# jtrefon/blt

Hardware: AMD Instinct MI355X
Metric: input GB/s tokenized (BPE) at 1/2/4/8 MI355X; % HBM roofline (higher is better)
Workload: dtype u8; 1 GPU; cfg3: 1024 MiB synthetic text per GPU, 50000-line merges, --chunksize 16MB; stream_bytes=1073741824, bytes_per_gpu=1073741824, chunk_size=16777216, merges=50000, parallelism=chunk-sharded x1, no collective

## Files before the change

blt_amd/_lib.py:

```python
from __future__ import annotations

import ctypes
import os
import re

_HERE = os.path.dirname(os.path.abspath(__file__))
LIB_PATH = os.environ.get("BLT_LIB_PATH") or os.path.join(_HERE, "libblt_bpe.so")
HEADER_PATH = os.path.join(os.path.dirname(_HERE), "include", "blt_bpe.h")

BLT_E_NOT_FOUND = -2
BLT_E_INVALID_DATA = -74
BLT_E_INVALID_INPUT = -22
BLT_E_NOSPC = -28
BLT_E_NOMEM = -12
BLT_E_IO = -5
BLT_E_NODEV = -19

ERROR_KINDS = {
    BLT_E_NOT_FOUND: "NotFound",
    BLT_E_INVALID_DATA: "InvalidData",
    BLT_E_INVALID_INPUT: "InvalidInput",
    BLT_E_NOSPC: "NoSpace",
    BLT_E_NOMEM: "OutOfMemory",
    BLT_E_IO: "Other",
    BLT_E_NODEV: "NoDevice",
}


class BltError(OSError):

    def __init__(self, code: int, message: str):
        super().__init__(-code, message)
        self.code = code
        self.kind = ERROR_KINDS.get(code, "Other")
        self.message = message

    def __str__(self):
        return self.message


_lib = None

_u16p = ctypes.POINTER(ctypes.c_uint16)
_u64p = ctypes.POINTER(ctypes.c_uint64)
_szp = ctypes.POINTER(ctypes.c_size_t)
_vp = ctypes.c_void_p

class RunConfig(ctypes.Structure):
    _fields_ = [("input_path", ctypes.c_char_p), ("output_path", ctypes.c_char_p), ("bpe", ctypes.c_void_p),
                ("passthrough", ctypes.c_int), ("content_token", ctypes.c_uint32), ("threads", ctypes.c_uint64),
                ("chunk_size", ctypes.c_uint64), ("n_gpus", ctypes.c_int)]


_SIGNATURES = {
    "blt_version": (ctypes.c_char_p, []),
    "blt_last_error": (ctypes.c_char_p, []),
    "blt_load_bpe_merges": (ctypes.c_int, [ctypes.c_char_p, _u16p, _u16p, _u16p, ctypes.c_size_t, _szp]),
    "blt_parse_chunk_size": (ctypes.c_int, [ctypes.c_char_p, _u64p]),
    "blt_effective_chunk_size": (ctypes.c_uint64, [ctypes.c_int, ctypes.c_uint64, ctypes.c_uint64, ctypes.c_uint32]),
    "blt_determine_thread_count": (ctypes.c_uint64, [ctypes.c_int, ctypes.c_uint64]),
    "blt_bpe_create": (ctypes.c_int, [_u16p, _u16p, _u16p, ctypes.c_size_t, ctypes.c_uint32, ctypes.POINTER(_vp)]),
    "blt_bpe_create_from_file": (ctypes.c_int, [ctypes.c_char_p, ctypes.POINTER(_vp)]),
    "blt_bpe_destroy": (None, [_vp]),
    "blt_bpe_info": (ctypes.c_int, [_vp, _szp, ctypes.POINTER(ctypes.c_int)]),
    "blt_bpe_clear_error": (ctypes.c_int, [_vp]),
    "blt_run_tokenizer": (ctypes.c_int, [ctypes.POINTER(RunConfig)]),
    "blt_bpe_process_chunk": (ctypes.c_int, [_vp, _vp, ctypes.c_size_t, _vp, ctypes.c_size_t, _szp]),
    "blt_bpe_process_chunks": (ctypes.c_int, [_vp, _vp, ctypes.c_size_t, ctypes.c_size_t, ctypes.c_int, _vp,
                                              ctypes.c_size_t, _szp, _vp]),
    "blt_basic_process_chunk": (ctypes.c_int, [_vp, ctypes.c_size_t, _vp, ctypes.c_size_t, _szp]),
    "blt_bpe_workspace_size": (ctypes.c_size_t, [_vp, ctypes.c_uint64, ctypes.c_uint64]),
    "blt_bpe_encode_device": (ctypes.c_int, [_vp, _vp, ctypes.c_uint64, ctypes.c_uint64, _vp, _vp, _vp,
                                             ctypes.c_size_t, _vp, _u64p]),
    "blt_bpe_encode_device_ex": (ctypes.c_int, [_vp, _vp, ctypes.c_uint64, ctypes.c_uint64, _vp, _vp, _vp,
                                                ctypes.c_size_t, _vp, _u64p, ctypes.c_uint32]),
    "blt_bpe_workspace_reset": (ctypes.c_int, [_vp, _vp, ctypes.c_uint64, ctypes.c_uint64, _vp]),
    "blt_bpe_check_workspace": (ctypes.c_int, [_vp, _vp]),
    "blt_basic_encode_device": (ctypes.c_int, [_vp, ctypes.c_uint64, _vp, _vp]),
}

_DEBUG_SIGNATURES = {
    "blt_debug_inject_device_error": (ctypes.c_int, [_vp, _vp, _vp]),
    "blt_debug_set_tile_record": (None, [_vp]),
    "blt_debug_set_inject": (ctypes.c_uint32, [ctypes.c_uint32]),
    "blt_debug_last_u16_passes": (ctypes.c_uint32, []),
    "blt_debug_last_scan_passes": (ctypes.c_uint32, []),
    "blt_debug_set_u16_chain": (ctypes.c_int, [ctypes.c_int]),
    "blt_debug_set_fused_only": (ctypes.c_int, [ctypes.c_int]),
    "blt_debug_set_shared_contexts": (None, [ctypes.c_int]),
    "blt_debug_set_pin_ring": (ctypes.c_int, [ctypes.c_int]),
    "blt_debug_set_fused": (None, [ctypes.c_int]),
    "blt_debug_last_fused": (ctypes.c_uint32, []),
    "blt_debug_byte_mode": (ctypes.c_int, [_vp]),
    "blt_debug_chain_depth": (ctypes.c_uint32, [_vp]),
    "blt_debug_set_finish": (ctypes.c_int, [ctypes.c_int]),
    "blt_debug_set_sparse": (ctypes.c_int, [ctypes.c_int]),
    "blt_debug_last_sparse": (ctypes.c_uint32, []),
    "blt_debug_set_sparse_cap": (ctypes.c_uint32, [ctypes.c_uint32]),
    "blt_debug_available_cpus": (ctypes.c_uint64, [ctypes.c_char_p, ctypes.c_char_p, ctypes.c_uint64]),
}


def header_symbols():
    with open(HEADER_PATH) as f:
        text = f.read()
    return sorted(set(re.findall(r"\b(blt_[a-z0-9_]+)\s*\(", text)))


def _share_torch_runtime():
    if os.environ.get("BLT_STANDALONE_HIP") == "1":
        return
    try:
        import torch
        import torch.cuda
        libdir = os.path.join(os.path.dirname(torch.__file__), "lib")
        hip = os.path.join(libdir, "libamdhip64.so")
        if os.path.exists(hip):
            ctypes.CDLL(hip, mode=ctypes.RTLD_GLOBAL)
    except ImportError:
        pass


def lib():
    global _lib
    if _lib is None:
        if not os.path.exists(LIB_PATH):
            raise RuntimeError(f"{LIB_PATH} is not built: run `make` (or __graft_entry__.build())")
        _share_torch_runtime()
        L = ctypes.CDLL(LIB_PATH)
        for name, (res, args) in list(_SIGNATURES.items()) + list(_DEBUG_SIGNATURES.items()):
            try:
                fn = getattr(L, name)
            except AttributeError:
                if name in _DEBUG_SIGNATURES:
                    continue
                raise
            fn.restype = res
            fn.argtypes = args
        _lib = L
    return _lib


def check(rc: int) -> None:
    if rc != 0:
        msg = lib().blt_last_error().decode("utf-8", "replace")
        raise BltError(rc, msg)
```

blt_amd/csrc/blt_host.cpp:

```cpp
#include <errno.h>
#include <fcntl.h>
#include <sched.h>
#include <hip/hip_runtime.h>
#include <stdarg.h>
#include <stdint.h>
#include <stdio.h>
#include <string.h>
#include <unistd.h>

#include <algorithm>
#include <atomic>
#include <condition_variable>
#include <memory>
#include <mutex>
#include <string>
#include <thread>
#include <unordered_map>
#include <unordered_set>
#include <vector>

#include "../../include/blt_bpe.h"
#include "bpe_kernels.h"

namespace {
// ... 346 lines not shown
        is_comp[kv.first >> 16] = 1;
        is_comp[kv.first & 0xFFFF] = 1;
    }
    for (int t = 0; t < 65536 && h->single_pass; ++t)
        if (is_value[t] && is_comp[t]) h->single_pass = false;
    if (!h->single_pass) h->chain_depth = chain_depth(map);

    std::vector<uint8_t> used(65536, 0);
    size_t byte_pairs = 0;
    for (const auto& kv : map)
        if ((kv.first >> 16) < 256 && (kv.first & 0xFFFF) < 256) { used[kv.second] = 1; ++byte_pairs; }
    if (byte_pairs == 65536) {
        h->sentinel = 0x10000u;
    } else {
        uint32_t s = 0xFFFF;
        while (used[s]) --s;
        h->sentinel = s;
    }
    h->dense.assign(65536, (uint16_t)(h->sentinel & 0xFFFF));
    for (const auto& kv : map) {
        const uint32_t a = kv.first >> 16, b = kv.first & 0xFFFF;
        if (a < 256 && b < 256) h->dense[blt::dense_index(a, b)] = kv.second;
    }
    auto bswap = [](uint32_t v) { return (uint16_t)(((v & 0xFF) << 8) | ((v >> 8) & 0xFF)); };
    bool hi_merge = true, self_valued = false, byte_keys = true;
    std::vector<uint8_t> hi_used(256, 0);
    for (const auto& kv : map) {
        const uint32_t a = kv.first >> 16, b = kv.first & 0xFFFF;
        if (a < 256 && b < 256) {
            if (a == b) h->byte_self_pair = true;
            if (kv.second == a) self_valued = true;
            if (kv.second < 256) hi_merge = false;
            hi_used[kv.second >> 8] = 1;
        } else {
            byte_keys = false;
        }
    }
    h->allmerge = byte_pairs == 65536;
    if (hi_merge) {
        h->byte_mode = 0;
    } else if (!self_valued || h->allmerge) {
        h->byte_mode = 1;
    } else {
        h->byte_mode = -1;
        for (uint32_t m = 1; m < 256 && h->byte_mode < 0; ++m)
            if (!hi_used[m]) { h->byte_mode = 2; h->mark = m; }
    }
    h->live_first = !h->single_pass && byte_keys && h->byte_mode > 0;
    h->self_ne.assign(blt::kSelfEntries, 0);
    for (uint32_t a = 0; a < 256; ++a)
        for (uint32_t b = 0; b < 256; ++b) h->self_ne[blt::self_index(a, b)] = (uint16_t)a;
    for (const auto& kv : map) {
        const uint32_t a = kv.first >> 16, b = kv.first & 0xFFFF;
        if (a < 256 && b < 256)
            h->self_ne[blt::self_index(a, b)] = (h->byte_mode == 2 && kv.second == a) ? (uint16_t)((h->mark << 8) | a)
                                                                                     : kv.second;
    }
    h->self_be.resize(blt::kSelfEntries);
    for (uint32_t i = 0; i < blt::kSelfEntries; ++i) h->self_be[i] = bswap(h->self_ne[i]);
    if (!h->single_pass && !build_buckets(map, is_comp, h.get())) return fail(BLT_E_NOMEM, "cannot place the merge map in a hash table");
    *out = h.release();
    return 0;
}

int current_device(int* dev) {
    int count = 0;
    if (hipGetDeviceCount(&count) != hipSuccess || count < 1) return fail(BLT_E_NODEV, "no HIP device available");
    HIP_TRY(hipGetDevice(dev));
    if (*dev < 0 || *dev >= kMaxDevices) return fail(BLT_E_NODEV, "device index %d out of range", *dev);
    return 0;
}

void detail_stamp(const char* what) {
    static const bool on = getenv("BLT_CLI_TIMING") != nullptr;
    if (!on) return;
    static timespec t0 = [] { timespec t; clock_gettime(CLOCK_MONOTONIC, &t); return t; }();
    timespec t;
    clock_gettime(CLOCK_MONOTONIC, &t);
    fprintf(stderr, "blt timing: detail: %s %.4f s\n", what,
            (double)(t.tv_sec - t0.tv_sec) + 1e-9 * (double)(t.tv_nsec - t0.tv_nsec));
}

int device_tables(const blt_bpe* hc, int dev, DevTables** out, hipStream_t via = nullptr) {
    blt_bpe* h = const_cast<blt_bpe*>(hc);
    DevTables& t = h->dev[dev];
    std::call_once(t.once, [&]() {
        auto up256 = [](size_t x) { return (x + 255) & ~size_t(255); };
        const size_t b_dense = 65536 * sizeof(uint16_t), b_self = blt::kSelfEntries * sizeof(uint16_t);
        const size_t b_hash = h->hwords.size() * sizeof(uint32_t);
        const size_t o_ne = up256(b_dense), o_be = o_ne + up256(b_self), o_hash = o_be + up256(b_self);
        const size_t total = o_hash + up256(b_hash);
        std::vector<uint8_t> blob(total, 0);
        memcpy(blob.data(), h->dense.data(), b_dense);
        memcpy(blob.data() + o_ne, h->self_ne.data(), b_self);
        memcpy(blob.data() + o_be, h->self_be.data(), b_self);
        if (b_hash) memcpy(blob.data() + o_hash, h->hwords.data(), b_hash);
        hipStream_t us = via;
        uint8_t* base = nullptr;
        detail_stamp("tables: blob built");
        bool ok = us || hipStreamCreateWithFlags(&us, hipStreamNonBlocking) == hipSuccess;
        detail_stamp("tables: stream created");
        ok = ok && hipMalloc(&base, total) == hipSuccess;
        detail_stamp("tables: allocated");
        ok = ok && hipMemcpyAsync(base, blob.data(), total, hipMemcpyHostToDevice, us) == hipSuccess;
        detail_stamp("tables: copy issued");
        if (base) {
            t.dense = reinterpret_cast<uint16_t*>(base);
            t.self_ne = reinterpret_cast<uint16_t*>(base + o_ne);
            t.self_be = reinterpret_cast<uint16_t*>(base + o_be);
            if (b_hash) t.hbuckets = reinterpret_cast<uint2*>(base + o_hash);
        }
        ok = ok && hipStreamSynchronize(us) == hipSuccess;
        detail_stamp("tables: copied");
        if (us && us != via) (void)hipStreamDestroy(us);
        detail_stamp("tables: stream destroyed");
        if (!ok) t.status = BLT_E_IO;
    });
    if (t.status) return fail(t.status, "uploading merge tables to device %d failed", dev);
    *out = &t;
    return 0;
}

uint32_t* sticky_word(const blt_bpe* hc) {
    blt_bpe* h = const_cast<blt_bpe*>(hc);
    std::call_once(h->sticky_once, [h] {
        void* p = nullptr;
        if (hipHostMalloc(&p, 64, hipHostMallocMapped | hipHostMallocPortable | hipHostMallocCoherent) == hipSuccess) {
            memset(p, 0, 64);
            h->sticky.store(static_cast<uint32_t*>(p), std::memory_order_release);
        }
    });
    return h->sticky.load(std::memory_order_acquire);
}

int sticky_check(const blt_bpe* h) {
    const uint32_t* w = h->sticky.load(std::memory_order_acquire);
    if (w && __atomic_load_n(w, __ATOMIC_ACQUIRE))
        return fail(BLT_E_IO,
                    "a previous merge scan on this handle flagged a device error (look-back timeout, output range "
                    "or prefix invariant); its output is invalid (blt_bpe_clear_error resets the handle)");
    return 0;
}

uint64_t* g_debug_tiles = nullptr;
std::atomic<uint32_t> g_inject{0};
std::atomic<int> g_shared_contexts{0};
std::atomic<int> g_fused{1};
std::atomic<int> g_u16_chain{3};
std::atomic<int> g_fused_only{0};
constexpr uint32_t kEncodeNoFused = 1u << 31;
thread_local uint32_t t_last_u16_passes = 0;
thread_local uint32_t t_last_scan_passes = 0;
thread_local uint32_t t_last_fused = 0;

inline uint64_t up16(uint64_t x) { return (x + 15) & ~15ull; }
inline uint64_t up256(uint64_t x) { return (x + 255) & ~255ull; }

struct WsLayout {
    uint64_t ntiles, nchunks;
    uint64_t ctl, status, status2, total, off_a, off_b, cmap, cmap_stride, gstat, bytes, zero_bytes;
    uint64_t sp_holes, sp_bits0, sp_bits1, sp_bits2, sp_seeds0, sp_seeds1, sp_merges, sp_tileo, sp_status, sp_ctr, sp_ntiles,
        sp_slices;
    uint32_t sp_cap;
};
constexpr uint32_t kMaxBoundedPasses = 64;
inline bool chain_bounded(const blt_bpe* h) { return h->chain_depth && h->chain_depth <= kMaxBoundedPasses + 1; }
constexpr uint32_t kSparseMaxPasses = 250;
constexpr uint32_t kSparseCtrWords = 2 + 2 * (kSparseMaxPasses + 1);
constexpr uint64_t kChainBlock = 48;

WsLayout ws_layout(const blt_bpe* h, uint64_t n, uint64_t cs) {
    const bool single_pass = h->single_pass;
    WsLayout L{};
    const uint64_t tile = single_pass ? std::min<uint64_t>(blt::kTilePos, blt::kTilePosBytes)
                                      : std::min<uint64_t>(blt::kTilePosTok, blt::kTilePosBytes);
    L.ntiles = (n + tile - 1) / tile;
    L.nchunks = n ? (n + cs - 1) / cs : 0;
    L.ctl = 0;
    L.status = blt::kCtlBytes;
    L.zero_bytes = up16(blt::kCtlBytes + 8 * L.ntiles);
    L.total = L.zero_bytes;
    L.off_a = L.total + kChainBlock;
    L.off_b = L.off_a + up16(8 * (L.nchunks + 1));
    L.cmap = up256(L.off_b + up16(8 * (L.nchunks + 1)));
    L.cmap_stride = up256(8 * ((n + blt::kTokRange - 1) / blt::kTokRange));
    L.gstat = L.cmap + 3 * L.cmap_stride;
    L.status2 = up256(L.gstat + up16(8 * L.nchunks));
    L.bytes = single_pass ? L.cmap : L.status2 + up16(8 * L.ntiles);
    if (!single_pass && !chain_bounded(h) && n < (1ull << 32)) {
        const uint64_t bm = up16(4 * ((n + 31) / 32));
        const uint64_t cap = n / 16 + 4096;
        const uint64_t sptiles = (n + blt::kSparseTile - 1) / blt::kSparseTile;
        L.sp_cap = (uint32_t)cap;
        L.sp_ntiles = sptiles;
        L.sp_holes = up16(L.bytes);
        L.sp_bits0 = L.sp_holes + bm;
        L.sp_bits1 = L.sp_bits0 + bm;
        L.sp_bits2 = L.sp_bits1 + bm;
        L.sp_seeds0 = L.sp_bits2 + bm;
        L.sp_seeds1 = L.sp_seeds0 + up16(4 * cap);
        L.sp_merges = L.sp_seeds1 + up16(4 * cap);
        L.sp_tileo = L.sp_merges + up16(12 * cap);
        L.sp_status = L.sp_tileo + up16(4 * ((sptiles + 15) & ~15ull) + 16);
        L.sp_ctr = L.sp_status + up16(8 * sptiles);
        L.sp_slices = L.sp_ctr + up16(4ull * kSparseCtrWords) + 4ull * blt::kSparseSampleBlocks;
        L.bytes = L.sp_slices + 3ull * 4ull * blt::kSparseSlices;
    }
    return L;
}

int read_u64(const void* dptr, uint64_t* v, hipStream_t s) {
    HIP_TRY(hipMemcpyAsync(v, dptr, sizeof(uint64_t), hipMemcpyDeviceToHost, s));
    HIP_TRY(hipStreamSynchronize(s));
    return 0;
}

int ctl_error(const uint32_t* ctl) {
    if (ctl[1])
        return fail(BLT_E_IO,
                    "merge-scan device check failed (flags 0x%x: 1 look-back timeout, 2 output range, 4 prefix "
                    "invariant, 8 workgroup wait timeout, 16 chunk map, 32 workspace not zeroed for this size "
                    "(BLT_ENCODE_WORKSPACE_ZEROED past the last reset), 64 finish-kernel count invariant; first "
                    "at tile %u sub-tile %u, O=%llu, value=%llu, C=%u)",
                    ctl[1], ctl[2] ? ctl[2] - 1 : 0, ctl[3], (unsigned long long)ctl[4] | ((unsigned long long)ctl[5] << 32),
                    (unsigned long long)ctl[6] | ((unsigned long long)ctl[7] << 32), ctl[8]);
    return 0;
}

int check_ctl(uint8_t* ws, hipStream_t s) {
    uint32_t ctl[16] = {0};
    HIP_TRY(hipMemcpyAsync(ctl, ws, sizeof ctl, hipMemcpyDeviceToHost, s));
    HIP_TRY(hipStreamSynchronize(s));
    return ctl_error(ctl);
}

struct Chain {
    const uint64_t* n_in = nullptr;
    uint64_t* n_out = nullptr;
    uint32_t* done = nullptr;
    uint32_t pass_id = 0;
    bool next_scan = false;
};

struct U16Run {
    bool map_ready = false;
    bool st_ready = false;
    uint32_t par = 0;
    void reset() { map_ready = st_ready = false; }
};

int run_pass(const blt_bpe* h, const DevTables* t, int dev, hipStream_t s, uint8_t* ws, const WsLayout& L,
             const void* in, bool in_u16, uint64_t n, uint64_t cs, const uint64_t* cstart, void* out, bool be,
             uint64_t out_cap, uint64_t* chunk_off, bool ws_zeroed = false, const Chain* chain = nullptr,
             bool tok_scan = false, U16Run* run = nullptr) {
    const bool columnar = !in_u16 && cs >= blt::kMinChunkBytes && h->byte_mode >= 0 && be;
    const uint64_t tile = columnar ? blt::kTilePosBytes
                                   : in_u16 ? (tok_scan ? blt::kTilePosTok : blt::kTilePosU16) : blt::kTilePos;
    const uint64_t ntiles = (n + tile - 1) / tile;
    if (ntiles > 0xFFFFFFFFull) return fail(BLT_E_INVALID_INPUT, "input too large");
    if (!(g_u16_chain.load(std::memory_order_relaxed) & 1)) run = nullptr;
    const bool chained = in_u16 && chain && run;
    const bool merge_ready = chained && !tok_scan && run->st_ready;
    if (!ws_zeroed && !(in_u16 && tok_scan) && !merge_ready) {
        HIP_TRY(hipMemsetAsync(ws, 0, up16(blt::kCtlBytes + 8 * ntiles), s));
        if (chained) run->par = 0;
    }
    blt::PassParams p{};
    p.in = in;
    p.n = n;
    p.cs = cs;
    p.cstart = cstart;
    p.nchunks = L.nchunks;
    p.out = out;
    p.out_cap = out_cap;
    p.chunk_off = chunk_off;
    p.status = reinterpret_cast<uint64_t*>(ws + L.status);
    p.ctl = reinterpret_cast<uint32_t*>(ws + L.ctl);
    p.total = chain ? chain->n_out : reinterpret_cast<uint64_t*>(ws + L.total);
    if (chain) {
        p.n_dev = chain->n_in;
        p.done = chain->done;
        p.pass_id = chain->pass_id;
    }
    p.ntiles = (uint32_t)ntiles;
    p.sentinel = h->sentinel;
    p.dense = columnar ? (be ? t->self_be : t->self_ne) : t->dense;
    p.hbuckets = t->hbuckets;
    p.hmul1 = h->hmul1;
    p.hmul2 = h->hmul2;
    p.hshift = h->hshift;
    p.hbytes = (uint32_t)(h->hwords.size() * sizeof(uint32_t));
    p.hone = h->hone ? 1u : 0u;
    p.cs_magic = cs ? ~0ull / cs : 0;
    if (cs && cs % blt::kTilePosBytes == 0 && cs / blt::kTilePosBytes < (1ull << 31)) {
        p.cs_tiles = (uint32_t)(cs / blt::kTilePosBytes);
        p.cs_tiles_magic = p.cs_tiles > 1 ? (uint32_t)(0xFFFFFFFFull / p.cs_tiles) : 0u;
    }
    p.allm = h->allmerge ? 1u : 0u;
    p.mark = h->mark | (h->mark << 16);
    p.debug = g_debug_tiles;
    p.inject = g_inject.load(std::memory_order_relaxed);
    p.sticky = h->sticky.load(std::memory_order_acquire);
    const bool scan16 = in_u16 && tok_scan;
    const bool ready = scan16 && chained && run->map_ready;
    auto map = [&](uint32_t i) { return reinterpret_cast<uint64_t*>(ws + L.cmap + (uint64_t)(i % 3u) * L.cmap_stride); };
    const uint32_t r = chain ? chain->pass_id % 3u : 0u;
    if (scan16) p.cmap = map(r);
    if (chained) {
        const bool alt = run->par != 0;
        p.status = reinterpret_cast<uint64_t*>(ws + (alt ? L.status2 : L.status));
        p.status_zero = reinterpret_cast<uint64_t*>(ws + (alt ? L.status : L.status2));
        p.tick = alt ? blt::kCtlTickAlt : 0u;
        if (scan16 && chain->next_scan) {
            p.cmap_next = map(r + 1u);
            p.cmap_zero = map(r + 2u);
        }
        run->par ^= 1u;
        run->st_ready = true;
        run->map_ready = scan16 && chain->next_scan;
    }
    p.ws_check = (ws_zeroed && !in_u16 && !chain) ? 1u : 0u;
    if (columnar) HIP_TRY(blt::launch_scan_bytes(p, h->byte_mode, (chain && h->live_first) ? 1 : 0, dev, s));
    else if (scan16) {
        HIP_TRY(blt::launch_scan_tokens(p, ready ? 1 : 0, dev, s));
        ++t_last_scan_passes;
    }
    else HIP_TRY(blt::launch_merge_pass(p, in_u16 ? 1 : 0, be ? 1 : 0, dev, s));
    return 0;
}

int run_fused(const blt_bpe* h, const DevTables* t, int dev, hipStream_t s, uint8_t* ws, const WsLayout& L,
              const uint8_t* d_in, uint64_t n, uint64_t cs, uint8_t* d_out, uint64_t* chunk_off, uint64_t* total,
              uint32_t* done, uint32_t* fused_fail) {
    const uint64_t ntiles = (n + blt::kTilePosTok - 1) / blt::kTilePosTok;
    if (ntiles > 0xFFFFFFFFull) return fail(BLT_E_INVALID_INPUT, "input too large");
    blt::PassParams p{};
    p.in = d_in;
    p.n = n;
    p.cs = cs;
    p.nchunks = L.nchunks;
    p.out = d_out;
    p.out_cap = 2 * n;
    p.chunk_off = chunk_off;
    p.status = reinterpret_cast<uint64_t*>(ws + L.status);
    p.ctl = reinterpret_cast<uint32_t*>(ws + L.ctl);
    p.total = total;
    p.done = done;
    p.pass_id = 1;
    p.ntiles = (uint32_t)ntiles;
    p.hbuckets = t->hbuckets;
    p.hmul1 = h->hmul1;
    p.hmul2 = h->hmul2;
    p.hshift = h->hshift;
    p.hbytes = (uint32_t)(h->hwords.size() * sizeof(uint32_t));
    p.hone = h->hone ? 1u : 0u;
    p.cs_magic = ~0ull / cs;
    p.debug = g_debug_tiles;
    p.inject = g_inject.load(std::memory_order_relaxed);
    p.sticky = h->sticky.load(std::memory_order_acquire);
    p.fused_fail = fused_fail;
    HIP_TRY(blt::launch_scan_fused(p, dev, s));
    return 0;
}

int run_finish(const blt_bpe* h, const DevTables* t, int dev, hipStream_t s, uint8_t* ws, const WsLayout& L,
               uint8_t* d_out, uint32_t k, const uint64_t* off_in, uint64_t* off_out, uint64_t* total, uint32_t* done) {
    blt::PassParams p{};
    p.in = d_out;
    p.out = d_out;
    p.cstart = off_in;
    p.nchunks = L.nchunks;
    p.chunk_off = off_out;
    p.total = total;
    p.done = done;
    p.pass_id = k;
    p.status = reinterpret_cast<uint64_t*>(ws + L.gstat);
    p.ctl = reinterpret_cast<uint32_t*>(ws + L.ctl);
    p.hbuckets = t->hbuckets;
    p.hmul1 = h->hmul1;
    p.hmul2 = h->hmul2;
    p.hshift = h->hshift;
    p.hbytes = (uint32_t)(h->hwords.size() * sizeof(uint32_t));
    p.hone = h->hone ? 1u : 0u;
    p.sticky = h->sticky.load(std::memory_order_acquire);
    p.fin_gate = reinterpret_cast<uint32_t*>(ws + L.total + 32);
    p.debug = g_debug_tiles;
    p.inject = g_inject.load(std::memory_order_relaxed);
    HIP_TRY(blt::launch_finish(p, dev, s));
    return 0;
}

std::atomic<int> g_finish{1};

int chain_sticky(const blt_bpe* h, uint8_t* ws, const WsLayout& L, uint64_t passes) {
    if (!sticky_check(h)) return 0;
    const std::string sticky_msg = t_err;
    uint32_t ctl[16] = {0};
    if (hipMemcpy(ctl, ws + L.ctl, sizeof ctl, hipMemcpyDeviceToHost) == hipSuccess && ctl_error(ctl))
        return fail(BLT_E_IO, "%s; u16 passes 1..%llu: %s", sticky_msg.c_str(), (unsigned long long)passes, t_err.c_str());
    return fail(BLT_E_IO, "%s", sticky_msg.c_str());
}

std::atomic<int> g_sparse{1};
thread_local uint32_t t_last_sparse = 0;
std::atomic<uint32_t> g_sparse_cap{0};

struct SparseRun {
    bool gated = false;
    bool taken = false;
    bool complete = false;
    uint32_t passes = 0;
    uint32_t applied = 0;
    uint64_t rec[4] = {0, 0, 0, 0};
    bool rec_final = false;
};

struct SparseHost {
    uint32_t ctr[kSparseCtrWords];
    uint64_t rec[4];
};
struct SparseHostLease {
    const blt_bpe* h;
    SparseHost* p = nullptr;
    explicit SparseHostLease(const blt_bpe* hh) : h(hh) {
        {
            std::lock_guard<std::mutex> lk(h->sp_mu);
            if (!h->sp_free.empty()) {
                p = static_cast<SparseHost*>(h->sp_free.back());
                h->sp_free.pop_back();
            }
        }
        if (!p && hipHostMalloc(reinterpret_cast<void**>(&p), sizeof(SparseHost), hipHostMallocDefault) != hipSuccess)
            p = nullptr;
    }
    ~SparseHostLease() {
        if (!p) return;
        std::lock_guard<std::mutex> lk(h->sp_mu);
        h->sp_free.push_back(p);
    }
};

int run_sparse(const blt_bpe* h, const DevTables* t, int dev, hipStream_t s, uint8_t* ws, const WsLayout& L,
               uint8_t* d_out, const uint64_t* n_dev, uint64_t n_max, const uint64_t* gate, uint64_t k,
               const uint64_t* off_in, uint64_t* off_out, uint64_t* tot, SparseRun* r) {
    *r = SparseRun{};
    SparseHostLease lease(h);
    SparseHost* hb = lease.p;
    if (!L.sp_cap || !hb || n_max == 0 || n_max >= (1ull << 32)) return 0;
    if (dev < 0 || dev >= kMaxDevices) return fail(BLT_E_NODEV, "device index %d out of range", dev);
    uint32_t* ctr = reinterpret_cast<uint32_t*>(ws + L.sp_ctr);
    blt::SparseParams q{};
    q.tok = reinterpret_cast<uint16_t*>(d_out);
    q.n = n_max;
    q.n_dev = n_dev;
    q.gate = gate;
    q.holes = reinterpret_cast<uint32_t*>(ws + L.sp_holes);
    q.flags = ctr;
    q.merges = reinterpret_cast<uint32_t*>(ws + L.sp_merges);
    const uint32_t cap_over = g_sparse_cap.load(std::memory_order_relaxed);
    q.cap = cap_over ? std::min(cap_over, L.sp_cap) : L.sp_cap;
    q.hbuckets = t->hbuckets;
    q.hmul1 = h->hmul1;
    q.hmul2 = h->hmul2;
    q.hshift = h->hshift;
    q.hbytes = (uint32_t)(h->hwords.size() * sizeof(uint32_t));
    q.hone = h->hone ? 1u : 0u;
    q.coff_in = off_in;
    q.coff_out = off_out;
    q.nchunks = L.nchunks;
    q.tile_cnt = reinterpret_cast<uint32_t*>(ws + L.sp_tileo);
    q.super_cnt = q.tile_cnt + ((L.sp_ntiles + 15) & ~15ull);
    q.status = reinterpret_cast<uint64_t*>(ws + L.sp_status);
    q.zero = reinterpret_cast<uint4*>(ws + L.sp_tileo);
    q.zero16 = (uint32_t)(((L.sp_ctr - L.sp_tileo) + up16(4ull * kSparseCtrWords)) / 16);
    q.sample = reinterpret_cast<uint32_t*>(ws + L.sp_ctr + up16(4ull * kSparseCtrWords));
// ... 812 lines not shown
        mult = up(t[n - 2]) == 'K' ? 1024ull : 1024ull * 1024ull;
        if (num.empty()) return fail(BLT_E_INVALID_INPUT, "Number part missing for unit '%s'", t.substr(n - 2).c_str());
    } else if (digits) {
        num = t;
    } else {
        return fail(BLT_E_INVALID_INPUT,
                    "Invalid unit or format: '%s'. Number must be followed by KB, MB, or be raw bytes.", t.c_str());
    }
    uint64_t v = 0;
    if (*parse_unsigned(num, UINT64_MAX, &v)) return fail(BLT_E_INVALID_INPUT, "Invalid number: '%s'", num.c_str());
    *out = v * mult;
    return 0;
    )
}

uint64_t blt_effective_chunk_size(int has_cli, uint64_t cli, uint64_t threads, uint32_t memcap) {
    const uint64_t amin = 256ull * 1024, amax = 128ull * 1024 * 1024;
    const uint64_t dmin = 1024ull * 1024, dmax = 16ull * 1024 * 1024;
    if (has_cli) return std::min(std::max(cli, amin), amax);
    const uint64_t usable = (uint64_t)((double)total_ram_bytes() * ((double)memcap / 100.0));
    uint64_t c = usable / std::max<uint64_t>(threads, 1) / 4;
    c = std::min(std::max(c, dmin), dmax);
    return std::min(std::max(c, amin), amax);
}

uint64_t blt_determine_thread_count(int has_cli, uint64_t threads) {
    if (has_cli) return threads == 0 ? 1 : threads;
    return available_cpus();
}

int blt_bpe_create(const uint16_t* a, const uint16_t* b, const uint16_t* v, size_t n, uint32_t flags,
                   blt_bpe** out) {
    GUARDED(
    if (!out || (n && (!a || !b || !v))) return fail(BLT_E_INVALID_INPUT, "null argument");
    if (flags) return fail(BLT_E_INVALID_INPUT, "unknown flags 0x%x", flags);
    std::vector<uint32_t> keys(n);
    std::vector<uint16_t> vals(v, v + n);
    for (size_t i = 0; i < n; ++i) keys[i] = ((uint32_t)a[i] << 16) | b[i];
    return build_handle(keys, vals, out);
    )
}

int blt_bpe_create_from_file(const char* path, blt_bpe** out) {
    GUARDED(
    if (!path || !out) return fail(BLT_E_INVALID_INPUT, "null argument");
    std::vector<int32_t> table;
    if (int rc = load_merges_table(path, table)) {
        const std::string inner = t_err;
        return fail(rc, "Failed to load BPE merges: %s", inner.c_str());
    }
    std::vector<uint32_t> keys;
    std::vector<uint16_t> vals;
    for (uint32_t i = 0; i < 65536; ++i)
        if (table[i] >= 0) { keys.push_back(((i >> 8) << 16) | (i & 255)); vals.push_back((uint16_t)table[i]); }
    return build_handle(keys, vals, out);
    )
}

void blt_bpe_destroy(blt_bpe* h) {
    if (!h) return;
    for (int d = 0; d < kMaxDevices; ++d) {
        if (h->dev[d].dense) (void)hipFree(h->dev[d].dense);
    }
    if (uint32_t* w = h->sticky.load(std::memory_order_acquire)) (void)hipHostFree(w);
    for (void* p : h->sp_free) (void)hipHostFree(p);
    delete h;
}

int blt_bpe_info(const blt_bpe* h, size_t* n_entries, int* single_pass) {
    if (!h) return fail(BLT_E_INVALID_INPUT, "null handle");
    if (n_entries) *n_entries = h->n_entries;
    if (single_pass) *single_pass = h->single_pass ? 1 : 0;
    return 0;
}

int blt_bpe_clear_error(const blt_bpe* h) {
    if (!h) return fail(BLT_E_INVALID_INPUT, "null handle");
    uint32_t* w = h->sticky.load(std::memory_order_acquire);
    if (!w || !__atomic_exchange_n(w, 0u, __ATOMIC_ACQ_REL)) return 0;
    return fail(BLT_E_IO, "a merge scan on this handle had flagged a device error (now cleared)");
}

size_t blt_bpe_workspace_size(const blt_bpe* h, uint64_t n, uint64_t cs) {
    if (!h || cs == 0) return 0;
    return (size_t)ws_layout(h, n, cs).bytes;
}

int blt_bpe_encode_device(const blt_bpe* h, const uint8_t* d_in, uint64_t n, uint64_t cs, uint8_t* d_out,
                          uint64_t* d_chunk_off, void* d_ws, size_t ws_bytes, void* stream, uint64_t* out_tokens) {
    GUARDED(return encode_device(h, d_in, n, cs, d_out, d_chunk_off, d_ws, ws_bytes, (hipStream_t)stream, out_tokens);)
}

int blt_bpe_encode_device_ex(const blt_bpe* h, const uint8_t* d_in, uint64_t n, uint64_t cs, uint8_t* d_out,
                             uint64_t* d_chunk_off, void* d_ws, size_t ws_bytes, void* stream, uint64_t* out_tokens,
                             uint32_t flags) {
    if (flags & ~BLT_ENCODE_WORKSPACE_ZEROED) return fail(BLT_E_INVALID_INPUT, "unknown flags 0x%x", flags);
    GUARDED(
    return encode_device(h, d_in, n, cs, d_out, d_chunk_off, d_ws, ws_bytes, (hipStream_t)stream, out_tokens, flags);
    )
}

int blt_bpe_workspace_reset(const blt_bpe* h, void* d_ws, uint64_t n, uint64_t cs, void* stream) {
    if (!h || !d_ws || cs == 0) return fail(BLT_E_INVALID_INPUT, "bad argument");
    const WsLayout L = ws_layout(h, n, cs);
    HIP_TRY(hipMemsetAsync(d_ws, 0, L.zero_bytes, (hipStream_t)stream));
    if (L.ntiles <= 0xFFFFFFFFull)
        HIP_TRY(hipMemsetD32Async(static_cast<uint32_t*>(d_ws) + blt::kCtlCover, (int)(uint32_t)L.ntiles, 1,
                                  (hipStream_t)stream));
    return 0;
}

int blt_bpe_check_workspace(void* d_ws, void* stream) {
    if (!d_ws) return fail(BLT_E_INVALID_INPUT, "null workspace");
    hipStream_t s = (hipStream_t)stream;
    if (int rc = check_ctl(static_cast<uint8_t*>(d_ws), s)) {
        const std::string msg = t_err;
        uint32_t z[16] = {0};
        (void)hipMemcpyAsync(d_ws, z, sizeof z, hipMemcpyHostToDevice, s);
        (void)hipStreamSynchronize(s);
        return fail(rc, "%s", msg.c_str());
    }
    return 0;
}

int blt_debug_byte_mode(const blt_bpe* h) {
    if (!h) return -1;
    return (h->byte_mode & 0xFF) | (h->allmerge ? 0x100 : 0) | (h->live_first ? 0x200 : 0);
}

int blt_debug_set_finish(int on) { return g_finish.exchange(on ? 1 : 0); }
int blt_debug_set_sparse(int on) { return g_sparse.exchange(on ? 1 : 0); }
uint32_t blt_debug_last_sparse(void) { return t_last_sparse; }
uint32_t blt_debug_set_sparse_cap(uint32_t cap) { return g_sparse_cap.exchange(cap); }

uint32_t blt_debug_chain_depth(const blt_bpe* h) { return h ? h->chain_depth : 0; }

void blt_debug_set_shared_contexts(int on) { g_shared_contexts.store(on ? 1 : 0, std::memory_order_relaxed); }
int blt_debug_set_pin_ring(int on) { return g_pin_ring.exchange(on ? 1 : 0) > 0 ? 1 : 0; }

void blt_debug_set_fused(int on) { g_fused.store(on ? 1 : 0, std::memory_order_relaxed); }
int blt_debug_set_u16_chain(int bits) { return g_u16_chain.exchange(bits); }
int blt_debug_set_fused_only(int on) { return g_fused_only.exchange(on ? 1 : 0); }
uint32_t blt_debug_last_fused() { return t_last_fused; }

uint64_t blt_debug_available_cpus(const char* cgroup_root, const char* proc_cgroup, uint64_t logical) {
    return available_cpus(cgroup_root, proc_cgroup, logical);
}

void blt_debug_set_tile_record(uint64_t* d_buf) { g_debug_tiles = d_buf; }
uint32_t blt_debug_set_inject(uint32_t bits) { return g_inject.exchange(bits); }

uint32_t blt_debug_last_u16_passes(void) { return t_last_u16_passes; }
uint32_t blt_debug_last_scan_passes(void) { return t_last_scan_passes; }

int blt_debug_inject_device_error(const blt_bpe* h, void* d_ws, void* stream) {
    if (!h) return fail(BLT_E_INVALID_INPUT, "null handle");
    int dev;
    if (int rc = current_device(&dev)) return rc;
    uint32_t* w = sticky_word(h);
    if (!w) return fail(BLT_E_NOMEM, "cannot allocate the pinned error word");
    HIP_TRY(blt::launch_inject_error(static_cast<uint32_t*>(d_ws), w, (hipStream_t)stream));
    HIP_TRY(hipStreamSynchronize((hipStream_t)stream));
    return 0;
}

int blt_basic_encode_device(const uint8_t* d_in, uint64_t n, uint8_t* d_out, void* stream) {
    if ((!d_in || !d_out) && n) return fail(BLT_E_INVALID_INPUT, "null argument");
    if (((uintptr_t)d_in | (uintptr_t)d_out) & 15) return fail(BLT_E_INVALID_INPUT, "device buffers must be 16-byte aligned");
    int dev;
    if (int rc = current_device(&dev)) return rc;
    HIP_TRY(blt::launch_basic_expand(d_in, n, d_out, (hipStream_t)stream));
    return 0;
}

int blt_bpe_process_chunk(const blt_bpe* h, const uint8_t* in, size_t n, uint8_t* out, size_t out_cap,
                          size_t* out_len) {
    GUARDED(
    if (!h || !out_len || (n && (!in || !out))) return fail(BLT_E_INVALID_INPUT, "null argument");
    *out_len = 0;
    if (int rc = sticky_check(h)) return rc;
    if (n == 0) return 0;
    if (out_cap < 2 * (uint64_t)n) return fail(BLT_E_NOSPC, "out_cap %zu < 2 * n", out_cap);
    int dev;
    if (int rc = current_device(&dev)) return rc;
    uint64_t ntok = 0;
    if (int rc = encode_host_on(h, dev, in, n, n, out, &ntok, nullptr)) return rc;
    *out_len = 2 * ntok;
    return 0;
    )
}

int blt_basic_process_chunk(const uint8_t* in, size_t n, uint8_t* out, size_t out_cap, size_t* out_len) {
    GUARDED(
    if (!out_len || (n && (!in || !out))) return fail(BLT_E_INVALID_INPUT, "null argument");
    *out_len = 0;
    if (n == 0) return 0;
    if (out_cap < 2 * (uint64_t)n) return fail(BLT_E_NOSPC, "out_cap %zu < 2 * n", out_cap);
    int dev;
    if (int rc = current_device(&dev)) return rc;
    DevCtx* c = ctx_acquire(dev);
    if (!c) return fail(BLT_E_IO, "cannot create a HIP stream");
    CtxGuard guard{c};
    if (int rc = grow(&c->d_in, &c->in_cap, up16(n))) return rc;
    if (int rc = grow(&c->d_out, &c->out_cap, up16(2 * n))) return rc;
    HIP_TRY(hipMemcpyAsync(c->d_in, in, n, hipMemcpyHostToDevice, c->stream));
    HIP_TRY(blt::launch_basic_expand(c->d_in, n, c->d_out, c->stream));
    HIP_TRY(hipMemcpyAsync(out, c->d_out, 2 * n, hipMemcpyDeviceToHost, c->stream));
    HIP_TRY(hipStreamSynchronize(c->stream));
    *out_len = 2 * n;
    return 0;
    )
}

}

void blt_prewarm_chunks(const blt_bpe* h, uint64_t n, uint64_t cs, int n_gpus) try {
    if (!h || !n || !cs) return;
    const bool timing = getenv("BLT_CLI_TIMING") != nullptr;
    timespec t0;
    clock_gettime(CLOCK_MONOTONIC, &t0);
    auto stamp = [&](const char* what) {
        if (!timing) return;
        timespec t;
        clock_gettime(CLOCK_MONOTONIC, &t);
        fprintf(stderr, "blt timing: prewarm step: %s +%.4f s\n", what,
                (double)(t.tv_sec - t0.tv_sec) + 1e-9 * (double)(t.tv_nsec - t0.tv_nsec));
    };
    HostPlan plan;
    if (host_plan(h, n, cs, n_gpus, &plan) != 0) return;
    stamp("device count (runtime up)");
    const uint64_t g = plan.devs.size();
    const uint64_t nchunks = (n + cs - 1) / cs;
    const uint64_t share = (nchunks + g - 1) / g * cs;
    const uint64_t win = h->single_pass ? std::max<uint64_t>(cs, std::min<uint64_t>(kPipeWindow / cs * cs, share)) : share;
    const uint64_t per_ctx = ((n + win - 1) / win + g - 1) / g;
    const int slots = (int)std::min<uint64_t>(kPipeSlots, per_ctx);
    (void)sticky_word(h);
    detail_stamp("sticky word");
    for (uint64_t d = 0; d < g; ++d) {
        const int dev = plan.devs[d];
        if (hipSetDevice(dev) != hipSuccess) return;
        DevCtx* c = ctx_acquire(dev);
        if (!c) return;
        CtxGuard guard{c};
        stamp("context (streams)");
        DevTables* t;
        if (device_tables(h, dev, &t, c->stream) != 0) return;
        stamp("device tables");
        if (plan.multi) {
            if (slots > 0 && pipe_slot_ready(h, c->pipe[0], std::min(win, n), cs) != 0) return;
            stamp("pipeline slots");
            if (blt::launch_noop(c->pipe[0].stream) == hipSuccess) (void)hipStreamSynchronize(c->pipe[0].stream);
            stamp("code object loaded (first launch)");
        } else {
            const WsLayout L = ws_layout(h, n, cs);
            uint8_t* offp = reinterpret_cast<uint8_t*>(c->d_off);
            if (grow(&c->d_in, &c->in_cap, up16(n)) || grow(&c->d_out, &c->out_cap, up16(2 * n)) ||
                grow(&c->d_ws, &c->ws_cap, L.bytes) || grow(&offp, &c->off_cap, 8 * (L.nchunks + 1)))
                return;
            c->d_off = reinterpret_cast<uint64_t*>(offp);
        }
    }
    if (g == 1 && !plan.multi) (void)hipSetDevice(plan.devs[0]);
} catch (...) {
}

extern "C" {

int blt_bpe_process_chunks(const blt_bpe* h, const uint8_t* in, size_t n, size_t cs, int n_gpus, uint8_t* out,
                           size_t out_cap, size_t* out_len, uint64_t* chunk_out_len) {
    GUARDED(
    if (!h || !out_len || (n && (!in || !out))) return fail(BLT_E_INVALID_INPUT, "null argument");
    if (cs == 0) return fail(BLT_E_INVALID_INPUT, "chunk_size must be > 0");
    *out_len = 0;
    if (int rc = sticky_check(h)) return rc;
    if (n == 0) return 0;
    if (out_cap < 2 * (uint64_t)n) return fail(BLT_E_NOSPC, "out_cap %zu < 2 * n", out_cap);
    const uint64_t nchunks = (n + cs - 1) / cs;
    HostPlan plan;
    if (int rc = host_plan(h, n, cs, n_gpus, &plan)) return rc;
    uint64_t total = 0;
    std::vector<uint64_t> offs;
    if (!plan.multi) {
        if (int rc = encode_host_on(h, plan.devs[0], in, n, cs, out, &total, chunk_out_len ? &offs : nullptr)) return rc;
    } else {
        if (int rc = encode_host_multi(h, plan.devs, in, n, cs, out, &total, chunk_out_len ? &offs : nullptr)) return rc;
    }
    if (chunk_out_len)
        for (uint64_t k = 0; k < nchunks; ++k) chunk_out_len[k] = 2 * (offs[k + 1] - offs[k]);
    *out_len = 2 * total;
    return 0;
    )
}

}
```

blt_amd/csrc/bpe_kernels.h:

```cpp
#pragma once
#include <hip/hip_runtime.h>
#include <stdint.h>

namespace blt {

constexpr int kSub = 4;
constexpr uint64_t kTilePos = 4 * 512 * 16;
constexpr uint64_t kTilePosU16 = kTilePos;
constexpr uint64_t kTilePosTok = 32768;
constexpr uint64_t kTokRange = 1024;
constexpr uint64_t kTilePosBytes = 32768;
constexpr uint64_t kMinChunkBytes = 4096;
constexpr uint64_t kCtlBytes = 64;
constexpr uint32_t kCtlLeft = 15;
constexpr uint32_t kCtlTickAlt = 12;
constexpr uint32_t kCtlCover = 14;

struct PassParams {
    const void* in;
    uint64_t n;
    uint64_t cs;
    const uint64_t* cstart;
    uint64_t nchunks;
    void* out;
    uint64_t* chunk_off;
    uint64_t* status;
    uint32_t* ctl;
    uint64_t out_cap;
    uint64_t* total;
    uint32_t ntiles;
    uint32_t sentinel;
    const uint16_t* dense;
    const uint2* hbuckets;
    uint32_t hmul1, hmul2;
    uint32_t hshift;
    uint32_t hbytes;
    uint32_t hone;
    const uint64_t* n_dev;
    uint32_t* done;
    uint32_t pass_id;
    uint64_t* cmap;
    uint64_t* cmap_next;
    uint64_t* cmap_zero;
    uint64_t* status_zero;
    uint32_t tick;
    uint64_t cs_magic;
    uint32_t cs_tiles;
    uint32_t cs_tiles_magic;
    uint32_t allm;
    uint32_t mark;
    uint32_t* sticky;
    uint32_t* fin_gate;
    uint32_t ws_check;
    uint32_t* fused_fail;
    uint64_t* debug;
    uint32_t inject;
};
constexpr uint32_t kInjectFinish = 1u, kInjectScanTok = 2u, kInjectSparseMove = 4u;

hipError_t launch_merge_pass(const PassParams& p, int input_u16, int big_endian, int device, hipStream_t s);
hipError_t launch_scan_bytes(const PassParams& p, int mode, int live, int device, hipStream_t s);
constexpr uint32_t kDoneBytePass = 0x80000000u;
hipError_t launch_scan_tokens(const PassParams& p, int map_ready, int device, hipStream_t s);
hipError_t launch_scan_fused(const PassParams& p, int device, hipStream_t s);
hipError_t launch_finish(const PassParams& p, int device, hipStream_t s);
constexpr uint64_t kFinCapTokens = 16384;
constexpr uint32_t kFinMaxGroupChunks = 1024;
hipError_t launch_basic_expand(const uint8_t* in, uint64_t n, uint8_t* out, hipStream_t s);
hipError_t launch_chain_final(const uint64_t* tot, const uint32_t* done, const uint64_t* off1, uint64_t* chunk_off,
                              uint64_t nchunks, uint32_t k_last, uint64_t* tot_final, hipStream_t s);
struct SparseParams {
    uint16_t* tok;
    uint64_t n;
    const uint64_t* n_dev;
    const uint64_t* gate;
    const uint32_t* cond;
    uint32_t* holes;
    uint32_t* seeds_in;
    uint32_t* nseeds_in;
    const uint32_t* cnt_in;
    uint32_t* bits_in;
    uint32_t* seeds_out;
    uint32_t* nseeds_out;
    uint32_t* bits_out;
    uint32_t* bits_alt;
    uint32_t first_pass;
    uint32_t* merges;
    uint32_t* nmerges;
    uint32_t* cnt_seeds;
    uint32_t* cnt_merges;
    uint32_t slice;
    uint32_t nslices;
    uint32_t* flags;
    uint32_t cap;
    const uint2* hbuckets;
    uint32_t hmul1, hmul2, hshift;
    uint32_t hbytes, hone;
    const uint64_t* coff_in;
    uint64_t* coff_out;
    uint64_t nchunks;
    uint64_t* total;
    uint32_t* tile_cnt;
    uint32_t* super_cnt;
    uint64_t* status;
    uint32_t* ctl;
    uint32_t* sticky;
    uint32_t* sample;
    uint4* zero;
    uint32_t zero16;
    uint32_t inject;
};
constexpr uint64_t kSparseTile = 8192;
constexpr uint32_t kSparseSlices = 4096;
constexpr uint32_t kSparseSampleBlocks = 64;
constexpr uint32_t kSparseSample = kSparseSampleBlocks * 8192u;
hipError_t launch_sparse_detect(const SparseParams& q, hipStream_t s);
hipError_t launch_sparse_list(const SparseParams& q, hipStream_t s);
hipError_t launch_sparse_pass(const SparseParams& q, hipStream_t s);
hipError_t launch_sparse_compact(const SparseParams& q, const uint32_t* nseeds0, hipStream_t s);
hipError_t launch_noop(hipStream_t s);
hipError_t launch_inject_error(uint32_t* ctl, uint32_t* sticky, hipStream_t s);

inline uint32_t dense_index(uint32_t a, uint32_t b) { return (a << 8) | (b ^ ((a << 1) & 0xFEu)); }

constexpr uint32_t kSelfRow = 258;
constexpr uint32_t kSelfEntries = 256 * kSelfRow;
inline uint32_t self_index(uint32_t a, uint32_t b) { return a * kSelfRow + b; }

inline uint32_t bucket_of(uint32_t key, uint32_t mul, uint32_t shift) {
    return (uint32_t)((key & 0xFFFFu) * (mul & 0xFFFFu) + (key >> 16) * (mul >> 16)) >> shift;
}
constexpr uint32_t kHashLdsMax = 48u << 10;

}
```

blt_amd/csrc/bpe_kernels.hip:

```cpp
#include <hip/hip_runtime.h>
#include <stdint.h>

#include <stddef.h>

#include <atomic>
#include <mutex>
#include <unordered_map>

#include "bpe_kernels.h"

namespace blt {

constexpr int kThreads = 512;
constexpr int kWaves = kThreads / 64;
constexpr int kSeg = 16;
constexpr int kSubPos = kThreads * kSeg;
constexpr int kStageBytes = 2 * kSubPos + 32;
constexpr uint32_t kSpinTimeoutTicks = 20000000u;
constexpr uint32_t kSpinClockEvery = 64;
struct SpinClock {
    uint32_t t0 = 0;
    uint32_t n = 0;
    __device__ __forceinline__ bool expired() {
        if ((++n % kSpinClockEvery) != 0u) return false;
// ... 464 lines not shown
                }
                st_publish(p.status + T, st_incl(C == 1u ? co1 : co0, end));
                s_C = C; s_O = O;
                if (p.debug) {
                    uint64_t* d = p.debug + 4ull * T;
                    d[0] = O;
                    d[1] = ((uint64_t)C << 32) | how;
                    d[2] = ((uint64_t)tf.cnt1 << 32) | tf.cnt0;
                    d[3] = ((uint64_t)co1 << 32) | co0;
                }
                s_tfn[2] = tf.cnt0; s_tfn[3] = tf.cnt1;
                if (T == p.ntiles - 1) {
                    *p.total = end;
                    if (p.chunk_off) p.chunk_off[p.nchunks] = end;
                    if (!kDense && p.done && end == p.n) *p.done = p.pass_id;
                }
            }
        }
        __syncthreads();

        if (s_C > 1u) continue;
        const uint32_t C = s_C;
        const uint64_t O = s_O;
        const uint32_t tile_cnt = C ? s_tfn[3] : s_tfn[2];
#pragma unroll
        for (int j = 0; j < kSubT; ++j) {
            const uint64_t sub0 = tile0 + (uint64_t)j * kSubPos;
            const uint64_t pos = sub0 + (uint64_t)tid * kSeg;
            const int g = j * kWaves + wave;
            const uint32_t cg = s_gin[g][C];
            const uint32_t og = s_gin[g][2 + C];
            const uint32_t c = hasb[j] ? bco[j] : cg;
            const uint32_t lane_off = og + (cg ? (excl[j] >> 16) : (excl[j] & 0xFFFFu));
            const uint32_t sub_first = s_gin[j * kWaves][2 + C];
            const uint32_t sub_end = (j + 1 < kSubT) ? s_gin[(j + 1) * kWaves][2 + C] : tile_cnt;
            const uint64_t gb = 2ull * (O + sub_first), ge = 2ull * (O + sub_end);
            const uint64_t ab = gb & ~15ull;
            const uint32_t M = merges_for(mm[j], c);
            const uint32_t L = lands_for(M, c, valid[j]);
            uint16_t* st16 = reinterpret_cast<uint16_t*>(s_stage);
            uint32_t r = (uint32_t)((2ull * (O + lane_off) - ab) >> 1);
#pragma unroll
            for (int k = 0; k < 16; ++k) {
                if ((L >> k) & 1u) {
                    uint32_t v = (vals[j][k >> 1] >> (16 * (k & 1))) & 0xFFFFu;
                    if constexpr (kDense) {
                        const uint32_t tok = ((M >> k) & 1u) ? v : seg[j].at(k);
                        st16[r++] = (uint16_t)(kBE ? bswap16(tok) : tok);
                    } else {
                        st16[r++] = (uint16_t)(((M >> k) & 1u) ? v : seg[j].at(k));
                    }
                }
            }
            if (p.chunk_off && nb < (uint32_t)kThreads) {
                const uint32_t lo = (uint32_t)(pos - tile0);
                for (uint32_t a = bnd_lower(lo); a < nb; ++a) {
                    const uint32_t r = s_bnd[a];
                    if (r > lo + 15u) break;
                    const uint32_t before = __popc(L & ((1u << (r - lo)) - 1u));
                    p.chunk_off[bk0 + a] = O + lane_off + before;
                }
            } else if (p.chunk_off) {
                uint64_t kidx;
                uint64_t b = first_boundary(p, sub0 < p.n ? sub0 : p.n, kidx);
                while (b < p.n && b < sub0 + kSubPos) {
                    if (b >= pos && b < pos + 16 && kidx < p.nchunks) {
                        uint32_t before = __popc(L & ((1u << (uint32_t)(b - pos)) - 1u));
                        p.chunk_off[kidx] = O + lane_off + before;
                    }
                    b = next_boundary(p, kidx);
                    ++kidx;
                }
            }
            __syncthreads();
            if (ge > p.out_cap || gb > ge) {
                if (tid == 0) record_error(p, 2u, T, (uint32_t)j, O, ge, C);
                __syncthreads();
                continue;
            }
            const uint32_t nblk = (uint32_t)((ge - ab + 15) >> 4);
            const uint4* st4 = reinterpret_cast<const uint4*>(s_stage);
            for (uint32_t i = tid; i < nblk; i += kThreads) {
                const uint64_t B = ab + 16ull * i;
                if (B >= gb && B + 16 <= ge) {
                    *reinterpret_cast<uint4*>(out + B) = st4[i];
                } else {
                    for (int u = 0; u < 8; ++u) {
                        const uint64_t bb = B + 2ull * u;
                        if (bb >= gb && bb < ge) *reinterpret_cast<uint16_t*>(out + bb) = st16[(bb - ab) >> 1];
                    }
                }
            }
            __syncthreads();
        }
    }
    if constexpr (kDense) self_reset(p, p.ntiles, &s_ticket);
}

template <typename InT, bool kBE>
__global__ __launch_bounds__(kThreads) void merge_pass_kernel(PassParams p) {
    merge_pass_body<InT, kBE, false>(p);
}
template <bool kHashLds>
__global__ __launch_bounds__(kThreads) void merge_tokens_kernel(PassParams p) {
    merge_pass_body<uint16_t, true, kHashLds>(p);
}

namespace seg {

typedef unsigned short u16x2 __attribute__((ext_vector_type(2)));
typedef unsigned int u32x4 __attribute__((ext_vector_type(4)));
__device__ __forceinline__ uint32_t pk_shl1(uint32_t v) {
    const u16x2 r = __builtin_bit_cast(u16x2, v) << (u16x2){1, 1};
    return __builtin_bit_cast(uint32_t, r);
}
__device__ __forceinline__ uint32_t pk_add(uint32_t a, uint32_t b) {
    const u16x2 r = __builtin_bit_cast(u16x2, a) + __builtin_bit_cast(u16x2, b);
    return __builtin_bit_cast(uint32_t, r);
}
__device__ __forceinline__ uint32_t pk_mul(uint32_t a, uint32_t b) {
    const u16x2 r = __builtin_bit_cast(u16x2, a) * __builtin_bit_cast(u16x2, b);
    return __builtin_bit_cast(uint32_t, r);
}
__device__ __forceinline__ uint32_t pk_nz(uint32_t v) {
    uint32_t r;
    asm("v_pk_min_u16 %0, %1, %2" : "=v"(r) : "v"(v), "s"(0x00010001u));
    return r;
}

typedef __attribute__((address_space(3))) uint16_t lds_u16;
typedef uint32_t __attribute__((aligned(2))) u32_a2;
typedef __attribute__((address_space(3))) u32_a2 lds_u32_a2;
typedef __attribute__((address_space(3))) uint8_t lds_u8;
__device__ __forceinline__ uint32_t lds_addr(const void* p) {
    return (uint32_t)(uintptr_t)(const lds_u8*)(p);
}
__device__ __forceinline__ uint32_t tab_addr_lo(uint32_t t, uint32_t base) {
    uint32_t a;
    asm("v_mad_u32_u16 %0, %1, 2, %2" : "=v"(a) : "v"(t), "s"(base));
    return a;
}
__device__ __forceinline__ uint32_t tab_addr_hi(uint32_t t, uint32_t base) {
    uint32_t a;
    asm("v_mad_u32_u16 %0, %1, 2, %2 op_sel:[1,0,0,0]" : "=v"(a) : "v"(t), "s"(base));
    return a;
}
__device__ __forceinline__ void add2(uint32_t& a, uint32_t bit) {
    asm("v_lshl_add_u32 %0, %1, 1, %0" : "+v"(a) : "v"(bit));
}

constexpr int kThreads = 1024;
constexpr int kWaves = kThreads / 64;
constexpr int kS = 2;
constexpr int kLdPol = 2, kStPol = 2;
constexpr uint32_t kWavePos = 64u * 16u;
constexpr uint64_t kSubPos = (uint64_t)kWaves * kWavePos;
constexpr int kGroups = kS * kWaves;
constexpr int kStageWave = 1536;
constexpr int kLbWin = 1;
constexpr uint32_t kNone = 0xFFFFFFFFu;
static_assert(kSubPos * kS == kTilePosBytes, "tile geometry");
static_assert(kWavePos <= kMinChunkBytes, "at most one chunk end per wave sub-tile");
static_assert(kGroups <= 64, "one lane per group in the tile resolve");
static_assert(kStageWave % 16 == 0, "stage alignment");
static_assert((uint64_t)kS * kSubPos == kTilePosBytes, "tile = kS sub-tiles");

__device__ __forceinline__ uint32_t uni(uint32_t v) { return (uint32_t)__builtin_amdgcn_readfirstlane((int)v); }
__device__ __forceinline__ uint64_t uni64(uint64_t v) {
    return ((uint64_t)uni((uint32_t)(v >> 32)) << 32) | uni((uint32_t)v);
}

__device__ __forceinline__ __amdgpu_buffer_rsrc_t rsrc_at(const void* base, uint64_t left) {
    const uint32_t records = uni((uint32_t)(left > 0x7FFFFFFFull ? 0x7FFFFFFFull : left));
    const uint64_t addr = uni64((uint64_t)(uintptr_t)base);
    return __builtin_amdgcn_make_buffer_rsrc(reinterpret_cast<void*>((uintptr_t)addr), (short)0, (int)records,
                                             0x00020000);
}
__device__ __forceinline__ __amdgpu_buffer_rsrc_t rsrc(const uint8_t* in, uint64_t base, uint64_t n) {
    return rsrc_at(in + (base < n ? base : 0), base < n ? n - base : 0);
}

template <int kCtrl, int kRowMask = 0xF>
__device__ __forceinline__ uint32_t dpp0(uint32_t v) {
    return (uint32_t)__builtin_amdgcn_update_dpp(0, (int)v, kCtrl, kRowMask, 0xF, false);
}
__device__ __forceinline__ uint32_t wave_scan(uint32_t v) {
    v += dpp0<0x111>(v);
    v += dpp0<0x112>(v);
    v += dpp0<0x114>(v);
    v += dpp0<0x118>(v);
    v += dpp0<0x142, 0xA>(v);
    v += dpp0<0x143, 0xC>(v);
    return v;
}
__device__ __forceinline__ uint32_t lane_sel(uint64_t mask, uint32_t if0, uint32_t if1) {
    uint32_t r;
    asm("v_cndmask_b32_e64 %0, %1, %2, %3" : "=v"(r) : "v"(if0), "v"(if1), "s"(mask));
    return r;
}
__device__ __forceinline__ uint32_t lane_u32(uint32_t v, int i) {
    return (uint32_t)__builtin_amdgcn_readlane((int)v, i);
}

template <int NS>
struct TileStateT {
    uint32_t v[NS][8];
    uint32_t mv[NS];
    uint32_t ex[NS];
};
using TileState = TileStateT<kS>;

struct TInfo {
    uint32_t rn;
    uint32_t bge;
    uint64_t k0;
};

constexpr uint32_t kFarPos = 2u * (uint32_t)kTilePosBytes;
__device__ __forceinline__ TInfo tile_info(const PassParams& p, uint32_t T) {
    TInfo t;
    const uint64_t tile0 = (uint64_t)T * kTilePosBytes;
    const uint64_t left = p.n > tile0 ? p.n - tile0 : 0;
    t.rn = (uint32_t)(left > 0x7FFFFFFFull ? 0x7FFFFFFFull : left);
    if (p.cs_tiles) {
        const uint32_t d = p.cs_tiles;
        uint32_t q = d == 1u ? T : __umulhi(T, p.cs_tiles_magic);
        uint32_t r = T - q * d;
        if (r >= d) { q += 1u; r -= d; }
        if (r >= d) { q += 1u; r -= d; }
        const uint32_t left_tiles = r ? d - r : 0u;
        t.bge = left_tiles > 2u ? kFarPos : left_tiles * (uint32_t)kTilePosBytes;
        t.k0 = (uint64_t)q + (r ? 1u : 0u);
        return t;
    }
    const uint64_t cs = KARG(cs);
    uint64_t q = __umul64hi(tile0, KARG(cs_magic));
    uint64_t r = tile0 - q * cs;
    if (r >= cs) { q += 1; r -= cs; }
    if (r >= cs) { q += 1; r -= cs; }
    const uint64_t d = r ? cs - r : 0;
    t.bge = (uint32_t)(d > kFarPos ? kFarPos : d);
    t.k0 = q + (r ? 1u : 0u);
    return t;
}

template <int NS>
__device__ __forceinline__ void lane_wave_fns(const uint32_t (&m)[NS], uint32_t wave, int lane, TileStateT<NS>& st,
                                              uint32_t (*wfn)[4], uint32_t wlive = 0u) {
    uint64_t wnonid[NS], wcmask[NS];
    uint32_t wincl[NS];
#pragma unroll
    for (int j = 0; j < NS; ++j) wnonid[j] = __ballot(m[j] != 0xFFFFu);
#pragma unroll
    for (int j = 0; j < NS; ++j) {
#ifndef BLT_NO_DENSE_FNS
        if (wnonid[j] == 0) {
            st.ex[j] = (uint32_t)lane * 0x00080008u | 0x80000000u;
            wcmask[j] = 0;
            wincl[j] = 0x02000200u;
            continue;
        }
#endif
        const uint32_t vm = st.mv[j] >> 16;
        const uint32_t mc = (m[j] & ~1u) | (m[j] << 16);
        const uint32_t sst = mc & ~pk_shl1(mc);
        const uint32_t rodd = mc & ~pk_add(mc, sst & 0xAAAAAAAAu);
        const uint32_t M = (mc & ~rodd & 0x55555555u) | (rodd & 0xAAAAAAAAu);
        const uint32_t L = ~(pk_shl1(M) | 1u) & (vm | (vm << 16));
        const uint32_t cnt0 = __popc(L & 0xFFFFu), cnt1 = __popc(L >> 16);
        const uint64_t nonid = wnonid[j];
        const uint64_t cmask = __ballot(((M >> 31) & 1u) == 0u);
        const uint64_t D = cmask & nonid, Mi = ~nonid, A = D << 1;
        const uint64_t Y = ((Mi + A) ^ Mi ^ A) | A;
        const uint64_t F = nonid ? ((nonid & (0ull - nonid)) << 1) - 1ull : ~0ull;
        const uint64_t CI0 = Y, CI1 = Y | F;
        const uint32_t packed = lane_sel(CI0, cnt0, cnt1) | (lane_sel(CI1, cnt0, cnt1) << 16);
        const uint32_t incl = wave_scan(packed);
        st.ex[j] = (incl - packed) | lane_sel(CI0, 0u, 0x8000u) | lane_sel(CI1, 0u, 0x80000000u);
        wcmask[j] = cmask;
        wincl[j] = incl;
    }
    if (lane == 63) {
#pragma unroll
        for (int j = 0; j < NS; ++j) {
            const uint32_t g = (uint32_t)j * kWaves + wave;
            const uint64_t nonid = wnonid[j];
            wfn[g][0] = (nonid == 0) | (wlive << 1);
            wfn[g][1] = nonid ? (uint32_t)((wcmask[j] >> (63 - __clzll(nonid))) & 1ull) : 0u;
            wfn[g][2] = wincl[j] & 0xFFFFu;
            wfn[g][3] = wincl[j] >> 16;
        }
    }
}

template <bool kBE, int kMode, bool kLive>
__device__ __forceinline__ void phase1_tile(uint32_t tab, const uint32_t (&x)[kS][4], const uint32_t (&nxt)[kS],
                                            const TInfo& ti, uint32_t cs32, uint32_t wave, int lane,
                                            TileState& st, uint32_t (*wfn)[4], uint32_t allm, uint32_t mark,
                                            uint64_t* sub = nullptr) {
    static_assert(kBE, "the byte pass writes big-endian tokens");
    static_assert(kMode >= 0 && kMode <= 2 && !(kLive && kMode == 0), "phase-1 mode");
    uint32_t m[kS];
#pragma unroll
    for (int j = 0; j < kS; ++j) {
        const uint32_t nbw = (uint32_t)__builtin_amdgcn_update_dpp((int)nxt[j], (int)x[j][0], 0x130, 0xF, 0xF, false);
#pragma unroll
        for (int h = 0; h < 8; ++h) {
            uint32_t va, vb;
#pragma unroll
            for (int e = 0; e < 2; ++e) {
                const int k = 2 * h + e;
                const uint32_t lo = x[j][k >> 2], hi = (k >> 2) < 3 ? x[j][(k >> 2) + 1] : nbw;
                const uint32_t sel = 0x0C000C00u | ((uint32_t)((k & 3) + 1) << 16) | (uint32_t)(k & 3);
                const uint32_t pr = __builtin_amdgcn_perm(hi, lo, sel);
                const uint32_t addr = __builtin_amdgcn_udot2(__builtin_bit_cast(u16x2, pr),
                                                             (u16x2){(unsigned short)(2 * kSelfRow), 2}, tab, false);
                const uint32_t v = *(const lds_u16*)(uintptr_t)addr;
                if (e == 0) va = v; else vb = v;
            }
            st.v[j][h] = __builtin_amdgcn_perm(vb, va, 0x05040100u);
        }
        uint32_t m32 = 0;
#pragma unroll
        for (int h = 0; h < 8; ++h) {
            uint32_t d;
            if (kMode == 0) {
                d = st.v[j][h] & 0x00FF00FFu;
            } else {
                const uint32_t xw = x[j][h >> 1];
                const uint32_t self = __builtin_amdgcn_perm(xw, xw, (h & 1) ? 0x030C020Cu : 0x010C000Cu);
                d = st.v[j][h] ^ self;
                if (kMode == 2) {
                    const uint32_t keep = pk_nz((st.v[j][h] ^ mark) & 0x00FF00FFu);
                    st.v[j][h] &= pk_mul(keep, 0x00FF00FFu) | 0xFF00FF00u;
                }
            }
            m32 |= pk_nz(d) << (2 * h);
        }
        if (allm) m32 = 0x7FFF7FFFu;
        m[j] = (m32 & 0xFFFFu) | (m32 >> 15);
    }
    uint32_t bnext = ti.bge;
#pragma unroll
    for (int j = 0; j < kS; ++j) {
        const uint32_t wrel = (uint32_t)j * (uint32_t)kSubPos + wave * kWavePos;
        while (bnext <= wrel) bnext += cs32;
        const uint32_t rem = ti.rn > wrel ? ti.rn - wrel : 0u;
        const bool has_end = bnext - 1u - wrel < kWavePos;
        if (rem <= kWavePos || has_end) {
            const uint32_t l16 = lane16_here();
            const int32_t r = (int32_t)(rem > 2u * kWavePos ? 2u * kWavePos : rem) - (int32_t)l16;
            const uint32_t vmask = r >= 16 ? 0xFFFFu : (r <= 0 ? 0u : ((1u << r) - 1u));
            uint32_t mm = m[j] & ((vmask >> 1) | (r > 16 ? 0x8000u : 0u));
            uint32_t forced = (r >= 1 && r <= 16) ? (1u << (r - 1)) : 0u;
            if (has_end) {
                const uint32_t e = bnext - 1u - wrel - l16;
                if (e < 16u) { mm &= ~(1u << e); forced |= 1u << e; }
            }
            if (__ballot(forced != 0)) {
#pragma unroll
                for (int h = 0; h < 8; ++h) {
                    const uint32_t xw = x[j][h >> 1];
                    const uint32_t raw = __builtin_amdgcn_perm(xw, xw, kBE ? ((h & 1) ? 0x030C020Cu : 0x010C000Cu)
                                                                           : ((h & 1) ? 0x0C030C02u : 0x0C010C00u));
                    const uint32_t fm = (((forced >> (2 * h)) & 1u) ? 0x0000FFFFu : 0u) |
                                        (((forced >> (2 * h + 1)) & 1u) ? 0xFFFF0000u : 0u);
                    st.v[j][h] = (st.v[j][h] & ~fm) | (raw & fm);
                }
            }
            m[j] = mm;
            st.mv[j] = mm | (vmask << 16);
        } else {
            st.mv[j] = m[j] | 0xFFFF0000u;
        }
    }
    uint32_t wlive = 0;
    if (kLive) {
        uint32_t lv = 0;
#pragma unroll
        for (int j = 0; j < kS; ++j) {
            uint32_t low32 = 0;
#pragma unroll
            for (int h = 0; h < 8; ++h) low32 |= (pk_nz(st.v[j][h] & 0x00FF00FFu) ^ 0x00010001u) << (2 * h);
            lv |= m[j] & ((low32 & 0xFFFFu) | (low32 >> 15));
        }
        wlive = __ballot(lv != 0u) != 0 ? 1u : 0u;
    }
    if (sub) {
        asm volatile("s_waitcnt lgkmcnt(0)" ::: "memory");
        sub[0] = __builtin_amdgcn_s_memtime();
    }
    lane_wave_fns<kS>(m, wave, lane, st, wfn, wlive);
    if (sub) {
        asm volatile("s_waitcnt lgkmcnt(0)" ::: "memory");
        sub[1] = __builtin_amdgcn_s_memtime();
    }
}

template <int NG = kGroups, bool kLive = false, bool kFresh = false>
__device__ __forceinline__ void resolve_tile(const PassParams& p, uint32_t T, int lane_arg, const uint32_t (*wfn)[4],
                                             uint32_t (*gin)[4], uint32_t* tfn) {
    const int lane = kFresh ? (int)(lane16_here() >> 4) : lane_arg;
    uint32_t gi = 1, gco = 0, g0 = 0, g1 = 0;
    if (lane < NG) { gi = wfn[lane][0]; gco = wfn[lane][1]; g0 = wfn[lane][2]; g1 = wfn[lane][3]; }
    const uint32_t tlive = kLive ? (__ballot((gi >> 1) & 1u) != 0) : 0u;
    if (kLive) gi &= 1u;
    const uint64_t nonid = __ballot(!gi);
    const uint64_t cmask = __ballot(gco);
    const uint64_t below = nonid & ((1ull << (uint32_t)lane) - 1ull);
    const uint32_t hb = below != 0;
    const uint32_t bc = hb ? (uint32_t)((cmask >> (63 - __clzll(below))) & 1ull) : 0u;
    const uint32_t cin0 = hb ? bc : 0u, cin1 = hb ? bc : 1u;
    uint32_t exc0, exc1, tot0, tot1;
    if constexpr ((uint64_t)NG * kWavePos < 65536u) {
        const uint32_t my = (cin0 ? g1 : g0) | ((cin1 ? g1 : g0) << 16);
        const uint32_t inc = wave_scan(my);
        const uint32_t exc = inc - my;
        exc0 = exc & 0xFFFFu; exc1 = exc >> 16;
        const uint32_t tot = lane_u32(inc, 63);
        tot0 = tot & 0xFFFFu; tot1 = tot >> 16;
    } else {
        const uint32_t my0 = cin0 ? g1 : g0, my1 = cin1 ? g1 : g0;
        const uint32_t inc0 = wave_scan(my0), inc1 = wave_scan(my1);
        exc0 = inc0 - my0; exc1 = inc1 - my1;
        tot0 = lane_u32(inc0, 63); tot1 = lane_u32(inc1, 63);
    }
    if (lane < NG) {
        gin[lane][0] = cin0;
        gin[lane][1] = cin1;
        gin[lane][2] = exc0;
        gin[lane][3] = exc1;
    }
    const uint32_t tident = nonid == 0;
    const uint32_t tcout = nonid ? (uint32_t)((cmask >> (63 - __clzll(nonid))) & 1ull) : 0u;
    const uint32_t co0 = tident ? 0u : tcout, co1 = tident ? 1u : tcout;
    if (lane == 0) {
        tfn[0] = co0 | (tlive << 1); tfn[1] = co1; tfn[2] = tot0; tfn[3] = tot1;
        st_publish(p.status + T, T == 0 ? st_incl(co1, tot1) | (tlive ? kStLiveIncl : 0ull)
                                        : st_agg(co0, co1, tot0, tot1) | (tlive ? kStLiveAgg : 0ull));
    }
}

template <bool kFresh = false>
__device__ __forceinline__ void lb_issue(const PassParams& p, int64_t k, int lane, uint64_t (&s)[kLbWin]) {
    if constexpr (kFresh) {
        const int32_t l = (int32_t)(lane16_here() >> 4);
#pragma unroll
        for (int q = 0; q < kLbWin; ++q) {
            const int32_t idx = (int32_t)k - l - 64 * q;
            s[q] = idx >= 0 ? st_read(p.status + (uint32_t)idx) : st_incl(1u, 0ull);
        }
    } else {
#pragma unroll
        for (int q = 0; q < kLbWin; ++q) {
            const int64_t idx = k - lane - 64 * q;
            s[q] = idx >= 0 ? st_read(p.status + idx) : st_incl(1u, 0ull);
        }
    }
}

template <bool kFresh = false>
__device__ __forceinline__ uint32_t win_apply(uint64_t s, int lim, int lane_arg, uint32_t c, uint64_t& tot,
                                              uint32_t& live) {
    const int lane = lane_arg;
    const bool in = lane < lim;
    live |= __ballot(in && (s & kStLiveAgg) != 0) != 0;
    const uint32_t hi = (uint32_t)(s >> 32), lo = (uint32_t)s;
    const uint32_t co0 = (hi >> 28) & 1u;
    const bool ident = ((hi >> 28) & 3u) == 2u;
    const uint64_t inm = __ballot(in);
    const uint64_t nonid = __ballot(in && !ident);
    const uint64_t comask = __ballot(in && co0);
    uint32_t cin;
    if (nonid == 0) {
        cin = c;
    } else if (nonid == inm) {
        const uint32_t up = (uint32_t)__builtin_amdgcn_update_dpp((int)co0, (int)co0, 0x130, 0xF, 0xF, false);
        cin = lane + 1 < lim ? up : c;
    } else {
        const uint64_t older = nonid & ~((~0ull) >> (63 - lane));
        cin = older ? (uint32_t)((comask >> __builtin_ctzll(older)) & 1ull) : c;
    }
    const uint32_t cnt = in ? (cin ? __builtin_amdgcn_alignbit(hi, lo, 30) & 0x1FFFFFFFu : lo & 0x3FFFFFFFu) : 0u;
    const uint32_t scan = wave_scan(cnt);
    tot += lane_u32(scan, 63);
    return nonid ? (uint32_t)((comask >> __builtin_ctzll(nonid)) & 1ull) : c;
}

struct TileFn {
    uint32_t co0, co1;
    uint64_t t0, t1;
};

template <bool kFresh = false>
__device__ void lb_finish(const PassParams& p, uint32_t Tp, int lane, uint64_t (&s)[kLbWin], uint32_t& C,
                          uint64_t& O, uint32_t& how, uint32_t& spins, uint32_t& live, uint32_t* bad_out = nullptr) {
    TileFn acc = {0u, 1u, 0ull, 0ull};
    int64_t k = (int64_t)Tp - 1;
    uint32_t rounds = 0;
    SpinClock clk;
    for (;;) {
        int qs = -1, f = 64;
        bool ready = true;
#pragma unroll
        for (int q = 0; q < kLbWin; ++q) {
            const uint32_t flag = (uint32_t)(s[q] >> 62);
            const uint64_t inc = __ballot(flag == 2u), rdy = __ballot(flag != 0u);
            if (qs < 0) {
                if (inc) {
                    f = __builtin_ctzll(inc);
                    const uint64_t need = (~0ull) >> (63 - f);
                    if ((rdy & need) != need) ready = false;
                    qs = q;
                } else if (rdy != ~0ull) {
                    ready = false;
                }
            }
        }
        if (!ready && spins == 0 && bad_out) {
            uint32_t d = 0;
#pragma unroll
            for (int q = kLbWin - 1; q >= 0; --q) {
                const uint64_t rdy = __ballot((uint32_t)(s[q] >> 62) != 0u);
                if (rdy != ~0ull) d = 64u * (uint32_t)q + (uint32_t)__builtin_ctzll(~rdy) + 1u;
            }
            *bad_out = d;
        }
        if (!ready) {
            ++spins;
            if (clk.expired()) {
                if (lane == 0) flag_error(p.ctl, KARG(sticky), 1u);
                C = 2u; O = 0ull;
                return;
            }
            __builtin_amdgcn_s_sleep(1);
            lb_issue<kFresh>(p, k, lane, s);
            continue;
        }
        if (qs < 0) {
            TileFn w;
#pragma unroll
            for (int h = 0; h < 2; ++h) {
                uint32_t c = (uint32_t)h;
                uint64_t t = 0;
#pragma unroll
// ... 31 lines not shown
}

__device__ __forceinline__ uint32_t funnel(uint32_t hi, uint32_t lo, uint32_t r) {
    return r ? __builtin_amdgcn_alignbyte(hi, lo, 2) : lo;
}
__device__ __forceinline__ u32x4 block_of(const u32x4& a, const u32x4& b, uint32_t d, uint32_t r) {
    u32x4 o;
    if (d == 0) {
        o[0] = funnel(a[1], a[0], r); o[1] = funnel(a[2], a[1], r); o[2] = funnel(a[3], a[2], r); o[3] = funnel(b[0], a[3], r);
    } else if (d == 1) {
        o[0] = funnel(a[2], a[1], r); o[1] = funnel(a[3], a[2], r); o[2] = funnel(b[0], a[3], r); o[3] = funnel(b[1], b[0], r);
    } else if (d == 2) {
        o[0] = funnel(a[3], a[2], r); o[1] = funnel(b[0], a[3], r); o[2] = funnel(b[1], b[0], r); o[3] = funnel(b[2], b[1], r);
    } else {
        o[0] = funnel(b[0], a[3], r); o[1] = funnel(b[1], b[0], r); o[2] = funnel(b[2], b[1], r); o[3] = funnel(b[3], b[2], r);
    }
    return o;
}
__device__ __forceinline__ void emit_dense(const uint32_t (&v)[8], uint32_t c, uint32_t rg, __amdgpu_buffer_rsrc_t ro,
                                           uint32_t ab, int lane) {
    const uint32_t sel = c ? 0x05040100u : 0x07060302u;
    u32x4 P;
#pragma unroll
    for (int q = 0; q < 4; ++q) P[q] = __builtin_amdgcn_perm(v[2 * q + 1], v[2 * q], sel);
    const uint32_t o = ab + 16u * (uint32_t)lane;
    if (rg == 0) {
        __builtin_amdgcn_raw_buffer_store_b128(P, ro, (int)o, 0, kStPol);
        return;
    }
    u32x4 Q;
#pragma unroll
    for (int q = 0; q < 4; ++q)
        Q[q] = (uint32_t)__builtin_amdgcn_update_dpp((int)P[q], (int)P[q], 0x138, 0xF, 0xF, false);
    const uint32_t off = 16u - rg;
    if (lane != 0) __builtin_amdgcn_raw_buffer_store_b128(block_of(Q, P, off >> 2, off & 3u), ro, (int)o, 0, kStPol);
    if (lane == 0 || lane == 63) {
        const uint32_t h = 8u - (rg >> 1);
#pragma unroll
        for (int k = 0; k < 8; ++k) {
            const uint16_t tok = (uint16_t)(P[k >> 1] >> (16 * (k & 1)));
            if (lane == 0 && (uint32_t)k < h) __builtin_amdgcn_raw_buffer_store_b16(tok, ro, (int)(ab + rg + 2u * k), 0, 0);
            if (lane == 63 && (uint32_t)k >= h)
                __builtin_amdgcn_raw_buffer_store_b16(tok, ro, (int)(ab + 1024u + 2u * (k - h)), 0, 0);
        }
    }
}

__device__ __forceinline__ void stage_b16(const uint32_t (&v)[8], uint32_t L, uint32_t a) {
#pragma unroll
    for (int h = 0; h < 8; ++h) {
        const uint32_t tok = v[h];
        *(lds_u16*)(uintptr_t)a = (uint16_t)tok;
        add2(a, __builtin_amdgcn_ubfe(L, 2 * h, 1));
        if (h < 7 || ((L >> 15) & 1u)) *(lds_u16*)(uintptr_t)a = (uint16_t)(tok >> 16);
        if (h < 7) add2(a, __builtin_amdgcn_ubfe(L, 2 * h + 1, 1));
    }
}

__device__ __forceinline__ uint32_t stage_phys(uint32_t x) { return x + ((x >> 6) << 3); }
__device__ __forceinline__ void stage_b16_pad(const uint32_t (&v)[8], uint32_t L, uint8_t* arr, uint32_t x) {
#pragma unroll
    for (int h = 0; h < 8; ++h) {
        const uint32_t tok = v[h];
        *reinterpret_cast<uint16_t*>(arr + stage_phys(x)) = (uint16_t)tok;
        add2(x, __builtin_amdgcn_ubfe(L, 2 * h, 1));
        if (h < 7 || ((L >> 15) & 1u)) *reinterpret_cast<uint16_t*>(arr + stage_phys(x)) = (uint16_t)(tok >> 16);
        if (h < 7) add2(x, __builtin_amdgcn_ubfe(L, 2 * h + 1, 1));
    }
}

constexpr int kCopyBlk = (kStageWave + 1023) / 1024;
constexpr int kStageTok = 2112;
constexpr int kStageTokPhys = kStageTok / 64 * 72;
constexpr int kCopyBlkTok = (kStageTok + 1023) / 1024;
struct CopyPart {
    uint32_t abp;
    uint32_t rgp;
    uint32_t re;
};
template <int NB = kCopyBlk>
struct CopyData {
    u32x4 vb[NB];
    uint16_t vf;
};
constexpr uint32_t kOobOff = 0x80000000u;
template <int NB>
__device__ __forceinline__ void copy_read(const uint8_t* stg, const CopyPart& c, int lane, CopyData<NB>& d) {
    const uint32_t hend = ((c.rgp + 15u) & ~15u) < c.re ? ((c.rgp + 15u) & ~15u) : c.re;
    const uint32_t tbeg = (c.re & ~15u) > hend ? (c.re & ~15u) : hend;
    const uint32_t nfull = (tbeg - hend) >> 4;
    const uint32_t of = lane < 8 ? c.rgp + 2u * (uint32_t)lane : tbeg + 2u * (uint32_t)(lane - 8);
    const bool bf = lane < 16 && of < (lane < 8 ? hend : c.re);
    const uint8_t* sp = stg;
    {
#pragma unroll
        for (int q = 0; q < NB; ++q)
            d.vb[q] = *reinterpret_cast<const u32x4*>(sp + min(hend + 16u * lane + 1024u * q, (uint32_t)kStageWave - 16u));
        d.vf = reinterpret_cast<const uint16_t*>(sp)[min(of >> 1, (uint32_t)kStageWave / 2u - 1u)];
        return;
    }
#pragma unroll
    for (int q = 0; q < NB; ++q) {
        d.vb[q] = (u32x4){0u, 0u, 0u, 0u};
        if ((uint32_t)lane + 64u * q < nfull) d.vb[q] = *reinterpret_cast<const u32x4*>(sp + hend + 16u * lane + 1024u * q);
    }
    d.vf = bf ? reinterpret_cast<const uint16_t*>(sp)[of >> 1] : (uint16_t)0;
}
template <int NB>
__device__ __forceinline__ void copy_read_pad(const uint8_t* arr, uint32_t x0, const CopyPart& c, int lane, CopyData<NB>& d) {
    const uint32_t hend = ((c.rgp + 15u) & ~15u) < c.re ? ((c.rgp + 15u) & ~15u) : c.re;
    const uint32_t tbeg = (c.re & ~15u) > hend ? (c.re & ~15u) : hend;
    const uint32_t nfull = (tbeg - hend) >> 4;
    const uint32_t of = lane < 8 ? c.rgp + 2u * (uint32_t)lane : tbeg + 2u * (uint32_t)(lane - 8);
    const bool bf = lane < 16 && of < (lane < 8 ? hend : c.re);
#pragma unroll
    for (int q = 0; q < NB; ++q) {
        d.vb[q] = (u32x4){0u, 0u, 0u, 0u};
        if ((uint32_t)lane + 64u * q < nfull) {
            const uint8_t* b = arr + stage_phys(x0 + hend + 16u * lane + 1024u * q);
            const uint2 lo = *reinterpret_cast<const uint2*>(b), hi = *reinterpret_cast<const uint2*>(b + 8);
            d.vb[q] = (u32x4){lo.x, lo.y, hi.x, hi.y};
        }
    }
    d.vf = bf ? *reinterpret_cast<const uint16_t*>(arr + stage_phys(x0 + of)) : (uint16_t)0;
}
template <int NB, bool kOob = true>
__device__ __forceinline__ void copy_store(__amdgpu_buffer_rsrc_t ro, const CopyPart& c, int lane, const CopyData<NB>& d) {
    const uint32_t hend = ((c.rgp + 15u) & ~15u) < c.re ? ((c.rgp + 15u) & ~15u) : c.re;
    const uint32_t tbeg = (c.re & ~15u) > hend ? (c.re & ~15u) : hend;
    const uint32_t nfull = (tbeg - hend) >> 4;
    const uint32_t of = lane < 8 ? c.rgp + 2u * (uint32_t)lane : tbeg + 2u * (uint32_t)(lane - 8);
    const bool bf = lane < 16 && of < (lane < 8 ? hend : c.re);
    if (kOob) {
#pragma unroll
        for (int q = 0; q < NB; ++q) {
            const uint32_t o = (uint32_t)lane + 64u * q < nfull ? c.abp + hend + 16u * lane + 1024u * q : kOobOff;
            __builtin_amdgcn_raw_buffer_store_b128(d.vb[q], ro, (int)o, 0, kStPol);
        }
        __builtin_amdgcn_raw_buffer_store_b16(d.vf, ro, (int)(bf ? c.abp + of : kOobOff), 0, 0);
        return;
    }
#pragma unroll
    for (int q = 0; q < NB; ++q)
        if ((uint32_t)lane + 64u * q < nfull)
            __builtin_amdgcn_raw_buffer_store_b128(d.vb[q], ro, (int)(c.abp + hend + 16u * lane + 1024u * q), 0, kStPol);
    if (bf) __builtin_amdgcn_raw_buffer_store_b16(d.vf, ro, (int)(c.abp + of), 0, 0);
}

struct SparseRange {
    uint32_t L, lane_off;
    uint32_t gb, wcnt;
};

__device__ __forceinline__ void emit_tile(const PassParams& p, uint32_t Tp, const TInfo& ti, uint32_t cs32,
                                          uint32_t wave, int lane, const TileState& st, const uint32_t (*gin)[4],
                                          uint32_t C, uint64_t O, uint8_t* stg, bool has_coff) {
    uint8_t* out = reinterpret_cast<uint8_t*>(KARG(out));
    const uint64_t out_cap = KARG(out_cap);
    const uint64_t obase = (2ull * O) & ~15ull;
    const uint32_t orel = (uint32_t)(2ull * O - obase);
    const __amdgpu_buffer_rsrc_t ro = rsrc_at(out + obase, out_cap > obase ? out_cap - obase : 0);
    const uint32_t stg_lds = lds_addr(stg);
    uint32_t cnext = ti.bge;
    uint64_t kc = ti.k0;
    SparseRange sr[kS];
    bool sparse[kS];
#pragma unroll
    for (int j = 0; j < kS; ++j) {
        const uint32_t g = (uint32_t)j * kWaves + wave;
        const uint32_t wrel = (uint32_t)j * (uint32_t)kSubPos + wave * kWavePos;
        const uint32_t cg = uni(gin[g][C]);
        const uint32_t goff = uni(gin[g][2 + C]);
        const uint32_t gb = orel + 2u * goff;
        while (cnext < wrel) { cnext += cs32; ++kc; }
        const bool cstart = has_coff && cnext < ti.rn && cnext - wrel < kWavePos;
        sparse[j] = __ballot(st.mv[j] != 0xFFFFFFFFu) != 0;
        if (!sparse[j]) {
            if (cstart && lane == 0) KARG(chunk_off)[kc] = O + goff;
            emit_dense(st.v[j], cg, gb - (gb & ~15u), ro, gb & ~15u, lane);
            continue;
        }
        const uint32_t m = st.mv[j] & 0xFFFFu, vmask = st.mv[j] >> 16;
        const uint32_t c = __builtin_amdgcn_ubfe(st.ex[j], 16u * cg + 15u, 1);
        const uint32_t lane_off = __builtin_amdgcn_ubfe(st.ex[j], 16u * cg, 15);
        const uint32_t mc = c ? m : (m & ~1u);
        const uint32_t sst = mc & ~(mc << 1);
        const uint32_t rodd = mc & ~(mc + (sst & 0xAAAAu));
        const uint32_t M = (mc & ~rodd & 0x5555u) | (rodd & 0xAAAAu);
        const uint32_t L = ~((M << 1) | (c ^ 1u)) & vmask;
        if (cstart) {
            const uint32_t e = cnext - wrel - lane16_here();
            if (e < 16u) KARG(chunk_off)[kc] = O + goff + lane_off + __popc(L & ((1u << e) - 1u));
        }
        sr[j].L = L;
        sr[j].lane_off = lane_off;
        sr[j].gb = gb;
        sr[j].wcnt = uni(lane_u32(lane_off + __popc(L), 63));
    }
    auto fits = [&](int j) { return (sr[j].gb & 15u) + 2u * sr[j].wcnt <= (uint32_t)kStageWave; };
#pragma unroll
    for (int j = 0; j < kS; ++j) {
        if (!sparse[j]) continue;
        const uint32_t two = fits(j) ? 0u : 1u;
        const uint32_t off32 = two ? uni(lane_u32(sr[j].lane_off, 32)) : 0u;
        for (uint32_t part = 0; part <= two; ++part) {
            const uint32_t base = part ? off32 : 0u;
            const uint32_t cnt = two ? (part ? sr[j].wcnt - off32 : off32) : sr[j].wcnt;
            const uint32_t gbp = sr[j].gb + 2u * base;
            if (!two || ((uint32_t)lane >> 5) == part) {
                stage_b16(st.v[j], sr[j].L, stg_lds + (gbp & 15u) + 2u * (sr[j].lane_off - base));
            }
            const CopyPart cp = {gbp & ~15u, gbp & 15u, (gbp & 15u) + 2u * cnt};
            CopyData<> d;
            copy_read(stg, cp, lane, d);
            copy_store(ro, cp, lane, d);
        }
    }
}

__device__ __forceinline__ void load_tile(const PassParams& p, uint32_t Tn, uint32_t wave, int lane,
                                          uint32_t (&x)[kS][4], uint32_t (&nxt)[kS]) {
    const uint8_t* in = reinterpret_cast<const uint8_t*>(KARG(in));
    const uint64_t tile0 = (uint64_t)Tn * kTilePosBytes;
    const uint64_t left = p.n > tile0 ? p.n - tile0 : 0;
    const __amdgpu_buffer_rsrc_t r = rsrc_at(in + tile0, left);
    const __amdgpu_buffer_rsrc_t rd = rsrc_at(in + tile0, left & ~3ull);
    const uint32_t rn = (uint32_t)(left > 0x7FFFFFFFull ? 0x7FFFFFFFull : left);
#pragma unroll
    for (int j = 0; j < kS; ++j) {
        const uint32_t wrel = (uint32_t)j * (uint32_t)kSubPos + wave * kWavePos;
        const auto v = __builtin_amdgcn_raw_buffer_load_b128(rd, (int)wrel + 16 * lane, 0, kLdPol);
        x[j][0] = v[0]; x[j][1] = v[1]; x[j][2] = v[2]; x[j][3] = v[3];
        nxt[j] = (uint32_t)__builtin_amdgcn_raw_buffer_load_b32(rd, (int)(wrel + kWavePos), 0, 0);
    }
#pragma unroll
    for (int j = 0; j < kS; ++j) {
        const uint32_t wrel = (uint32_t)j * (uint32_t)kSubPos + wave * kWavePos;
        if (rn > wrel && rn - wrel < kWavePos + 16u) {
            nxt[j] = (uint32_t)__builtin_amdgcn_raw_buffer_load_b8(r, (int)(wrel + kWavePos), 0, 0);
#pragma unroll
            for (int q = 0; q < 4; ++q) {
                uint32_t d = 0;
#pragma unroll
                for (int b = 0; b < 4; ++b)
                    d |= (uint32_t)__builtin_amdgcn_raw_buffer_load_b8(r, (int)wrel + 16 * lane + 4 * q + b, 0, 0)
                         << (8 * b);
                x[j][q] = d;
            }
        }
    }
}

constexpr int kRing = 4;
#ifdef BLT_TIMING
constexpr bool kTiming = true;
#else
constexpr bool kTiming = false;
#endif
constexpr int kPrioP1Wave = kWaves / 2, kPrioP1 = 1;
constexpr int kPrioEmWave = 3 * kWaves / 4, kPrioEm = 2;
constexpr int kTkTid = 64;
__device__ __forceinline__ uint32_t lds_acquire(const uint32_t* f) {
    return __hip_atomic_load(const_cast<uint32_t*>(f), __ATOMIC_ACQUIRE, __HIP_MEMORY_SCOPE_WORKGROUP);
}
__device__ __forceinline__ void lds_release(uint32_t* f, uint32_t v) {
    __hip_atomic_store(f, v, __ATOMIC_RELEASE, __HIP_MEMORY_SCOPE_WORKGROUP);
}
__device__ __forceinline__ void wait_ge(const PassParams& p, const uint32_t* f, uint32_t v) {
    SpinClock clk;
    while (lds_acquire(f) < v) {
        if (clk.expired()) {
            if ((threadIdx.x & 63) == 0) flag_error(p.ctl, KARG(sticky), 8u);
            break;
        }
        __builtin_amdgcn_s_sleep(1);
    }
}

template <bool kBE, int kMode, bool kLive>
__global__ __launch_bounds__(kThreads) void scan_bytes_kernel(PassParams p) {
    __shared__ __attribute__((aligned(16))) uint16_t s_tab[kSelfEntries];
    __shared__ __attribute__((aligned(16))) uint8_t s_stage[kWaves][kStageWave];
    __shared__ __attribute__((aligned(16))) uint32_t s_wfn[kRing][kGroups][4];
    __shared__ uint32_t s_gin[kRing][kGroups][4];
    __shared__ uint32_t s_tfn[kRing][4];
    __shared__ uint64_t s_O[kRing];
    __shared__ uint32_t s_C[kRing];
    __shared__ uint32_t s_tk[kRing];
    __shared__ uint32_t s_p1cnt[kRing];
    __shared__ uint32_t s_rdone;
    __shared__ uint32_t s_lbdone;
    __shared__ uint32_t s_tkdone;

    const int tid = threadIdx.x;
    const int lane = tid & 63;
    const uint32_t wave = uni((uint32_t)tid >> 6);
    const uint64_t n = p.n;
    const uint32_t ntiles = p.ntiles;
    const uint32_t cs32 = (uint32_t)(p.cs > kFarPos ? kFarPos : p.cs);
    const uint32_t allm = uni(p.allm), mark = uni(p.mark);
    const bool has_coff = p.chunk_off != nullptr;

    const uint32_t cover = ws_cover(p);
    uint64_t* const wg_rec = (kTiming && p.debug) ? p.debug + (8ull + 8ull * kWaves) * p.ntiles + 4ull * blockIdx.x : nullptr;
    if (wg_rec && tid == 0) wg_rec[0] = __builtin_amdgcn_s_memrealtime();
    if (tid == 0) {
        s_tk[kRing - 2] = atomicAdd(p.ctl, 1u);
        s_tk[kRing - 1] = atomicAdd(p.ctl, 1u);
        for (int r = 0; r < kRing; ++r) s_p1cnt[r] = 0;
        s_rdone = 0; s_lbdone = 0; s_tkdone = 0;
    }
    {
        const uint4* src = reinterpret_cast<const uint4*>(p.dense);
        uint4* dst = reinterpret_cast<uint4*>(s_tab);
        constexpr int kUnits = (int)(kSelfEntries * 2 / 16);
        constexpr int kPer = (kUnits + kThreads - 1) / kThreads;
#pragma unroll
        for (int k = 0; k < kPer; ++k) {
            const int u0 = (int)wave * 64 + k * kThreads;
            if (k < kPer - 1 || u0 < kUnits)
                __builtin_amdgcn_global_load_lds(
                    (__attribute__((address_space(1))) void*)(src + u0 + lane),
                    (__attribute__((address_space(3))) void*)(dst + u0), 16, 0, 0);
        }
    }
    __syncthreads();
    if (wg_rec && tid == 0) wg_rec[1] = __builtin_amdgcn_s_memrealtime();
    const uint32_t tab = uni(lds_addr(s_tab));
    uint32_t T = uni(s_tk[kRing - 2]);
    uint32_t Tp = kNone;
    uint32_t Tq = uni(s_tk[kRing - 1]);
    if (ws_refused(p, ntiles, cover)) T = kNone;
    if (T >= ntiles || Tq >= ntiles) Tq = kNone;
    TInfo ti = {}, tip = {};
    if (T < ntiles) ti = tile_info(p, T);
    __syncthreads();

    uint32_t xa[kS][4], xb[kS][4];
    uint32_t na[kS], nb[kS];
    if (T < ntiles) load_tile(p, T, wave, lane, xa, na);
    TileState sa, sb;
    uint64_t lbs[kLbWin];
    uint32_t it = 0;

    auto step = [&](uint32_t (&x)[kS][4], uint32_t (&nxt)[kS], uint32_t (&xq)[kS][4], uint32_t (&nxtq)[kS],
                    TileState& sc, const TileState& sp) {
        const uint32_t slot = it & (kRing - 1), pslot = (it - 1) & (kRing - 1);
        uint64_t stamp[7], sub[2] = {0, 0};
        const bool stamping = kTiming && p.debug != nullptr;
        if (stamping) stamp[0] = __builtin_amdgcn_s_memtime();
        __builtin_amdgcn_s_waitcnt(0x0F70);
        if (stamping) stamp[1] = __builtin_amdgcn_s_memtime();
        if (Tq < ntiles) load_tile(p, Tq, wave, lane, xq, nxtq);
        uint32_t tk = kNone;
        if (tid == kTkTid && Tq < ntiles) tk = atomicAdd(p.ctl, 1u);
        asm volatile("" ::: "memory");

        bool lbw = wave == 0;
        if (T < ntiles) {
            if (wave >= (uint32_t)kPrioP1Wave) __builtin_amdgcn_s_setprio(kPrioP1);
            phase1_tile<kBE, kMode, kLive>(tab, x, nxt, ti, cs32, wave, lane, sc, s_wfn[slot], allm, mark,
                                           stamping ? sub : nullptr);
            __builtin_amdgcn_s_setprio(0);
            uint32_t old = 0;
            if (lane == 0)
                old = __hip_atomic_fetch_add(&s_p1cnt[slot], 1u, __ATOMIC_ACQ_REL, __HIP_MEMORY_SCOPE_WORKGROUP);
            old = uni(old);
            lbw = old == (uint32_t)kWaves * (it / kRing);
            if (old == (uint32_t)kWaves * (it / kRing + 1u) - 1u) {
                resolve_tile<kGroups, kLive, kMode != 0>(p, T, lane, s_wfn[slot], s_gin[slot], s_tfn[slot]);
                if (lane == 0) lds_release(&s_rdone, it + 1u);
                if (stamping && lane == 0) p.debug[4ull * ntiles + 4ull * T] = __builtin_amdgcn_s_memrealtime();
            }
        }
        if (stamping) stamp[2] = __builtin_amdgcn_s_memtime();

        if (lbw && Tp < ntiles) {
            uint32_t C = 1u, how = 0xFFFFu, spins = 0, bad = 0, live = 0;
            uint64_t O = 0ull;
            const bool lb = Tp > 0;
            if (lb) lb_issue<kMode != 0>(p, (int64_t)Tp - 1, lane, lbs);
            const uint64_t rt_snap = stamping ? __builtin_amdgcn_s_memrealtime() : 0;
            wait_ge(p, &s_rdone, it);
            const uint32_t tfl = uni(s_tfn[pslot][0]), tf1 = uni(s_tfn[pslot][1]);
            const uint32_t tf0 = tfl & 1u, tf2 = uni(s_tfn[pslot][2]), tf3 = uni(s_tfn[pslot][3]);
            if (lb) lb_finish<kMode != 0>(p, Tp, lane, lbs, C, O, how, spins, live, kTiming ? &bad : nullptr);
            live |= (tfl >> 1) & 1u;
            if (lane == 0) {
                const uint64_t end = O + (C == 1u ? tf3 : tf2);
                if (C > 1u || O > (uint64_t)Tp * kTilePosBytes || end > n) {
                    if (C <= 1u) record_error(p, 4u, Tp, 0xFFu, O, end, C);
                    O = 0; C = 2u;
                }
                s_C[pslot] = C;
                s_O[pslot] = O;
                lds_release(&s_lbdone, it + 1u);
                const uint64_t fin = C > 1u ? 0ull : O + (C ? tf3 : tf2);
                if (Tp > 0) st_publish(p.status + Tp, st_incl(C == 1u ? tf1 : tf0, fin) | (live ? kStLiveIncl : 0ull));
                if (2ull * fin > KARG(out_cap)) record_error(p, 2u, Tp, 0xFFu, O, fin, C);
                if (Tp == ntiles - 1) {
                    *KARG(total) = fin;
                    if (uint64_t* co = KARG(chunk_off)) co[KARG(nchunks)] = fin;
                    if (kLive && C <= 1u && (fin == n || !live))
                        if (uint32_t* dn = KARG(done)) *dn = kDoneBytePass;
                }
                if (kDebugRecord && p.debug) {
                    uint64_t* d = p.debug + 4ull * Tp;
                    d[0] = O;
                    d[1] = ((uint64_t)C << 32) | how;
                    d[2] = ((uint64_t)tf3 << 32) | tf2;
                    d[3] = ((uint64_t)tf1 << 32) | tf0;
                    if (kTiming) {
                        uint64_t* e = p.debug + 4ull * ntiles + 4ull * Tp;
                        e[3] = spins | ((uint64_t)bad << 32);
                        e[1] = (rt_snap & 0xFFFFFFFFull) | (__builtin_amdgcn_s_memrealtime() << 32);
                    }
                }
            }
        }

        if (stamping) stamp[3] = __builtin_amdgcn_s_memtime();
        if (Tp < ntiles) {
            wait_ge(p, &s_lbdone, it + 1u);
            if (stamping) stamp[4] = __builtin_amdgcn_s_memtime();
            if (wave >= (uint32_t)kPrioEmWave) __builtin_amdgcn_s_setprio(kPrioEm);
            const uint32_t Cp = uni(s_C[pslot]);
            if (Cp <= 1u)
                emit_tile(p, Tp, tip, cs32, wave, lane, sp, s_gin[pslot], Cp, uni64(s_O[pslot]), s_stage[wave], has_coff);
            __builtin_amdgcn_s_setprio(0);
        }
        if (stamping) stamp[5] = __builtin_amdgcn_s_memtime();
        if (stamping && Tp < ntiles && lane == 0) {
            stamp[6] = __builtin_amdgcn_s_memtime();
            uint64_t* w = p.debug + 8ull * ntiles + 8ull * ((uint64_t)Tp * kWaves + wave);
#pragma unroll
            for (int q = 0; q < 6; ++q) w[q] = stamp[q + 1] - stamp[q];
            w[6] = sub[0] ? sub[0] - stamp[1] : 0;
            w[7] = sub[0] ? sub[1] - sub[0] : 0;
        }
        if (stamping && tid == 0 && Tp < ntiles) {
            uint64_t* e = p.debug + 4ull * ntiles + 4ull * Tp;
            e[2] = __builtin_amdgcn_s_memtime();
        }
        if (tid == kTkTid) {
            s_tk[slot] = tk;
            lds_release(&s_tkdone, it + 1u);
        }
        uint32_t Tr = kNone;
        if (Tq < ntiles) {
            wait_ge(p, &s_tkdone, it + 1u);
            Tr = uni(s_tk[slot]);
            if (Tr >= ntiles) Tr = kNone;
        }
        tip = ti;
        if (Tq < ntiles) ti = tile_info(p, Tq);
        Tp = T;
        T = Tq;
        Tq = Tr;
        ++it;
    };
    for (;;) {
        if (!(T < ntiles || Tp < ntiles)) break;
        step(xa, na, xb, nb, sa, sb);
        if (!(T < ntiles || Tp < ntiles)) break;
        step(xb, nb, xa, na, sb, sa);
    }
    if (wg_rec && lane == 0)
        atomicMax(reinterpret_cast<unsigned long long*>(wg_rec + 2), (unsigned long long)__builtin_amdgcn_s_memrealtime());
    self_reset(p, ntiles, &s_tkdone);
}

constexpr int kSt = (int)(kTilePosTok / kTokRange) / kWaves;
constexpr uint32_t kSubTok = (uint32_t)kWaves * kWavePos;
constexpr uint32_t kTileTok = (uint32_t)kSt * kSubTok;
constexpr int kGroupsTok = kSt * kWaves;
static_assert(kTileTok == kTilePosTok && kWavePos == kTokRange, "token tile geometry");
static_assert(kGroupsTok <= 64 && kS * kWaves <= 64, "groups");

constexpr uint32_t kCmStart = 1u << 11, kCmEnd = 1u << 23;

__device__ __forceinline__ void cm_mark(const PassParams& p, uint64_t* m, uint64_t P, uint32_t c) {
    const uint64_t o1 = __hip_atomic_fetch_or(m + (P >> 10), (P & 1023u) | kCmStart | ((uint64_t)c << 32),
                                              __ATOMIC_RELAXED, __HIP_MEMORY_SCOPE_AGENT);
    uint64_t o2 = 0;
    if (c) o2 = __hip_atomic_fetch_or(m + ((P - 1) >> 10), (((P - 1) & 1023u) << 12) | kCmEnd, __ATOMIC_RELAXED,
                                      __HIP_MEMORY_SCOPE_AGENT);
    if ((o1 & kCmStart) || (o2 & kCmEnd)) flag_error(p.ctl, KARG(sticky), 16u);
}

__device__ __forceinline__ uint64_t token_count(const PassParams& p) {
    return p.n_dev ? __hip_atomic_load(const_cast<uint64_t*>(p.n_dev), __ATOMIC_RELAXED, __HIP_MEMORY_SCOPE_AGENT) : p.n;
}
__device__ __forceinline__ bool pass_done(const PassParams& p) {
    return p.done && __hip_atomic_load(p.done, __ATOMIC_RELAXED, __HIP_MEMORY_SCOPE_AGENT) != 0u;
}

__device__ __forceinline__ uint64_t cm_word(const uint64_t* cs, uint64_t nc, uint64_t lo, uint64_t hi, bool& bad) {
    uint64_t a = 0, b = nc;
    while (a < b) {
        const uint64_t mid = (a + b) >> 1;
        if (cs[mid] < lo) a = mid + 1; else b = mid;
    }
    uint64_t w = 0;
    if (a < nc && cs[a] < hi) {
        w |= (cs[a] - lo) | kCmStart | (a << 32);
        bad |= a + 1 < nc && cs[a + 1] < hi;
    }
    const uint64_t e = (a < nc && cs[a] == lo) ? a + 1 : a;
    if (e < nc && cs[e] <= hi) {
        w |= ((cs[e] - 1 - lo) << 12) | kCmEnd;
        bad |= e + 1 < nc && cs[e + 1] <= hi;
    }
    return w;
}

constexpr uint32_t kCmLds = 1024;
__global__ __launch_bounds__(256) void chunk_map_kernel(PassParams p) {
    __shared__ uint64_t s_cs[kCmLds];
    const bool done = pass_done(p);
    const uint64_t n = token_count(p);
    if (done) return;
    const uint64_t r = (uint64_t)blockIdx.x * 256u + threadIdx.x;
    if (r < (n + kTileTok - 1) / kTileTok) p.status[r] = 0ull;
    if (p.cmap_next && r < (n + kWavePos - 1) / kWavePos) p.cmap_next[r] = 0ull;
    if (r == 0) { p.ctl[p.tick] = 0u; p.ctl[kCtlCover] = 0u; }
    const uint64_t nc = p.nchunks;
    const bool in_lds = nc <= kCmLds;
    if ((uint64_t)blockIdx.x * 256u * kWavePos >= n) return;
    if (in_lds) {
        for (uint32_t i = threadIdx.x; i < nc; i += 256u) s_cs[i] = p.cstart[i];
        __syncthreads();
    }
    const uint64_t lo = r * kWavePos, hi = lo + kWavePos;
    if (lo >= n) return;
    bool bad = false;
    const uint64_t w = in_lds ? cm_word(s_cs, nc, lo, hi, bad) : cm_word(p.cstart, nc, lo, hi, bad);
    if (bad) flag_error(p.ctl, KARG(sticky), 16u);
    p.cmap[r] = w;
}

__device__ __forceinline__ void load_tok(const PassParams& p, uint64_t n, uint32_t Tn, uint32_t wave, int lane,
                                         uint32_t (&x)[kSt][8], uint32_t (&nxt)[kSt], uint32_t& cw) {
    const uint8_t* in = reinterpret_cast<const uint8_t*>(p.in);
    const uint64_t tile0 = (uint64_t)Tn * kTileTok;
    const uint64_t left = n > tile0 ? n - tile0 : 0;
    const __amdgpu_buffer_rsrc_t rd = rsrc_at(in + 2 * tile0, (2 * left) & ~3ull);
    const uint64_t r0 = (uint64_t)Tn * kGroupsTok, nr = (n + kWavePos - 1) / kWavePos;
    const __amdgpu_buffer_rsrc_t rm = rsrc_at(p.cmap + r0, nr > r0 ? 8 * (nr - r0) : 0);
#pragma unroll
    for (int j = 0; j < kSt; ++j) {
        const uint32_t wrel = (uint32_t)j * kSubTok + wave * kWavePos;
        const int o = 2 * (int)(wrel + 16u * (uint32_t)lane);
        const auto v0 = __builtin_amdgcn_raw_buffer_load_b128(rd, o, 0, kLdPol);
        const auto v1 = __builtin_amdgcn_raw_buffer_load_b128(rd, o + 16, 0, kLdPol);
        x[j][0] = v0[0]; x[j][1] = v0[1]; x[j][2] = v0[2]; x[j][3] = v0[3];
        x[j][4] = v1[0]; x[j][5] = v1[1]; x[j][6] = v1[2]; x[j][7] = v1[3];
        nxt[j] = (uint32_t)__builtin_amdgcn_raw_buffer_load_b32(rd, (int)(2 * (wrel + kWavePos)), 0, 0);
    }
    static_assert(kSt == 2, "chunk-map words: 4 dwords per wave");
    const uint32_t cl = (lane16_here() >> 4) & 3u;
    cw = (uint32_t)__builtin_amdgcn_raw_buffer_load_b32(rm, (int)(8u * ((cl >> 1) * (uint32_t)kWaves + wave) + 4u * (cl & 1u)), 0, 0);
    const uint32_t rn = (uint32_t)(left > 0x7FFFFFFFull ? 0x7FFFFFFFull : left);
#pragma unroll
    for (int j = 0; j < kSt; ++j) {
        const uint32_t wrel = (uint32_t)j * kSubTok + wave * kWavePos;
        if (rn > wrel && rn - wrel < kWavePos + 16u) {
            const __amdgpu_buffer_rsrc_t r = rsrc_at(in + 2 * tile0, 2 * left);
            const int o = 2 * (int)(wrel + 16u * (uint32_t)lane);
            nxt[j] = (uint32_t)__builtin_amdgcn_raw_buffer_load_b16(r, (int)(2 * (wrel + kWavePos)), 0, 0);
#pragma unroll
            for (int q = 0; q < 8; ++q)
                x[j][q] = (uint32_t)__builtin_amdgcn_raw_buffer_load_b16(r, o + 4 * q, 0, 0) |
                          ((uint32_t)__builtin_amdgcn_raw_buffer_load_b16(r, o + 4 * q + 2, 0, 0) << 16);
        }
    }
}

template <int kHash>
__device__ __forceinline__ uint32_t tok_get(const PassParams& p, uint32_t tab, uint32_t key) {
    typedef unsigned int u32x2 __attribute__((ext_vector_type(2)));
    typedef __attribute__((address_space(3))) u32x2 lds_u32x2;
    const uint32_t b1 = bucket_hash(key, p.hmul1, p.hshift);
    if constexpr (kHash == 2) {
        const u32x2 x = *(const lds_u32x2*)(uintptr_t)(tab + 8u * b1);
        return x[0] == key ? x[1] : 0u;
    }
    const uint32_t b2 = bucket_hash(key, p.hmul2, p.hshift);
    u32x2 x, y;
    if constexpr (kHash == 1) {
        x = *(const lds_u32x2*)(uintptr_t)(tab + 8u * b1);
        y = *(const lds_u32x2*)(uintptr_t)(tab + 8u * b2);
    } else {
        const u32x2* g = reinterpret_cast<const u32x2*>(p.hbuckets);
        x = g[b1];
        y = g[b2];
    }
    return (x[0] == key ? x[1] : 0u) | (y[0] == key ? y[1] : 0u);
}

template <int kHash>
__device__ __forceinline__ uint32_t phase1_tok(const PassParams& p, uint32_t tab, const uint32_t (&x)[8],
                                               uint32_t nxt, uint32_t rem, uint32_t cwl, int lane, int j,
                                               TileStateT<kSt>& st, uint32_t& live, bool next_ok = false) {
    const uint32_t nbw = (uint32_t)__builtin_amdgcn_update_dpp((int)nxt, (int)x[0], 0x130, 0xF, 0xF, false);
    uint32_t r[16];
#pragma unroll
    for (int k = 0; k < 16; ++k) {
        const int h = k >> 1;
        const uint32_t key = (k & 1) ? __builtin_amdgcn_alignbyte(h < 7 ? x[h + 1] : nbw, x[h], 2) : x[h];
        r[k] = tok_get<kHash>(p, tab, key);
    }
    uint32_t racc = 0;
#pragma unroll
    for (int k = 0; k < 16; k += 2) racc |= r[k] | r[k + 1];
    uint32_t lv = (racc >> 30) & 1u;
    uint32_t m32 = 0;
#pragma unroll
    for (int h = 0; h < 8; ++h) {
        const uint32_t R = __builtin_amdgcn_perm(r[2 * h + 1], r[2 * h], 0x05040100u);
        const uint32_t hit = __builtin_amdgcn_perm(r[2 * h + 1], r[2 * h], 0x0B0B0909u);
        st.v[j][h] = (hit & R) | (~hit & x[h]);
        m32 |= (hit & 0x00010001u) << (2 * h);
// ... 754 lines not shown
        if (ncnt > n || 2u * ncnt < n) {
            bad = 0xF2u;
            break;
        }
        const uint32_t cg = s_gin[wave][0];
        const uint32_t c = hasb ? bco : cg;
        const uint32_t lane_off = s_gin[wave][1] + (cg ? (excl >> 16) : (excl & 0xFFFFu));
        const uint32_t M = merges_for(m, c);
        const uint32_t L = lands_for(M, c, vmask);
        if (ncnt != n) {
            if (vmask) seg::stage_b16(v, L, seg::lds_addr(&s_tok[cur ^ 1][0]) + 2u * lane_off);
            if (nc > 1 && wave_on) {
                for (uint32_t a = a_lo > 0 ? a_lo - 1 : 0; a < nc; ++a) {
                    const uint32_t b = s_cpos[cur][a];
                    if (b >= pos0 + 16u) break;
                    if (b >= pos0) s_cpos[cur ^ 1][a] = lane_off + __popc(L & ((1u << (b - pos0)) - 1u));
                }
            }
            if (tid == 0) { s_cpos[cur ^ 1][0] = 0u; s_cpos[cur ^ 1][nc] = ncnt; }
        }
        __syncthreads();
        if (ncnt == n) break;
        cur ^= 1;
        n = ncnt;
    }
    if (!bad) {
        bool ok = true;
        for (uint32_t i = tid; i < nc; i += kFinThreads) ok = ok && s_cpos[cur][i] <= s_cpos[cur][i + 1];
        if (__syncthreads_or(!ok || s_cpos[cur][nc] != n)) bad = 0xF3u;
    }

    if (wave == 0) {
        uint32_t C = 1u, how = 0, spins = 0;
        uint64_t O = 0;
        const uint32_t cnt = bad ? (uint32_t)(nin64 < (1ull << 30) ? nin64 : (1ull << 30) - 1u) : n;
        if (g == 0) {
            if (lane == 0) st_publish(p.status, st_incl(1u, cnt));
        } else {
            if (lane == 0) st_publish(p.status + g, st_agg(1u, 1u, cnt, cnt));
            if (!bad) {
                fin_lookback(p, g, lane, C, O, how, spins);
                if (lane == 0) {
                    if (C > 1u || O > S) {
                        if (C <= 1u) record_error(p, 4u, (uint32_t)g, 0xFEu, O, n, C);
                        O = ~0ull;
                    } else {
                        st_publish(p.status + g, st_incl(1u, O + n));
                    }
                }
            }
        }
        if (bad) {
            if (lane == 0) record_error(p, kFinBadBit, (uint32_t)g, bad, S, bad == 0xF2u ? s_cnt : n, nc);
            O = ~0ull;
        }
        if (lane == 0) {
            s_O = O;
            if (p.debug) {
                uint64_t* d = p.debug + 16ull * g;
                d[0] = g; d[1] = S; d[2] = nin64; d[3] = n; d[4] = O;
                d[5] = C | ((uint64_t)how << 8) | ((uint64_t)spins << 32);
                d[6] = lmax | ((uint64_t)grp << 32); d[7] = nc | ((uint64_t)bad << 32);
                d[8] = g ? st_read(p.status + g - 1) : 0; d[9] = st_read(p.status);
                d[10] = st_read(p.status + g);
                d[11] = g >= 2 ? st_read(p.status + g - 2) : 0;
            }
        }
    }
    __syncthreads();
    const uint64_t O = s_O;
    if (O == ~0ull) continue;
    uint16_t* out = reinterpret_cast<uint16_t*>(p.out);
    for (uint32_t i = tid; i < n; i += kFinThreads) out[O + i] = s_tok[cur][i];
    for (uint32_t i = tid; i < nc; i += kFinThreads) p.chunk_off[c0 + i] = O + s_cpos[cur][i];
    if (c1 == p.nchunks && tid == 0) {
        p.chunk_off[p.nchunks] = O + n;
        *p.total = O + n;
        *p.done = p.pass_id;
    }
    }
}

__global__ void inject_error_kernel(uint32_t* ctl, uint32_t* sticky) {
    if (threadIdx.x == 0) flag_error(ctl, sticky, 1u);
}

struct GridCache {
    std::atomic<int> cus[64];
    std::atomic<int> occ[64][16];
};
static GridCache g_grid;
static int grid_for(uint32_t ntiles, int device, const void* fn, int threads, int kernel_id) {
    int cus = 0, occ = 0;
    if (device >= 0 && device < 64) {
        cus = g_grid.cus[device].load(std::memory_order_relaxed);
        occ = g_grid.occ[device][kernel_id].load(std::memory_order_relaxed);
    }
    if (!cus) {
        if (hipDeviceGetAttribute(&cus, hipDeviceAttributeMultiprocessorCount, device) != hipSuccess || cus < 1) cus = 1;
        if (device >= 0 && device < 64) g_grid.cus[device].store(cus, std::memory_order_relaxed);
    }
    if (!occ) {
        if (hipOccupancyMaxActiveBlocksPerMultiprocessor(&occ, fn, threads, 0) != hipSuccess || occ < 1) occ = 1;
        if (device >= 0 && device < 64) g_grid.occ[device][kernel_id].store(occ, std::memory_order_relaxed);
    }
    long long g = (long long)cus * occ;
    if (g > (long long)ntiles) g = ntiles;
    return (int)(g < 1 ? 1 : g);
}

static std::mutex g_grid_mu;
static std::unordered_map<uint64_t, int> g_grid_smem;
static int grid_for_smem(uint32_t ntiles, int device, const void* fn, int threads, size_t smem) {
    const uint64_t key = ((uint64_t)(uint32_t)device << 40) ^ ((uint64_t)(uintptr_t)fn << 20) ^ (uint64_t)smem;
    int g = 0;
    {
        std::lock_guard<std::mutex> lk(g_grid_mu);
        auto it = g_grid_smem.find(key);
        if (it != g_grid_smem.end()) g = it->second;
    }
    if (!g) {
        int cus = 0, occ = 0;
        if (hipDeviceGetAttribute(&cus, hipDeviceAttributeMultiprocessorCount, device) != hipSuccess || cus < 1) cus = 1;
        if (hipOccupancyMaxActiveBlocksPerMultiprocessor(&occ, fn, threads, smem) != hipSuccess || occ < 1) occ = 1;
        g = cus * occ;
        std::lock_guard<std::mutex> lk(g_grid_mu);
        g_grid_smem[key] = g;
    }
    if ((uint64_t)g > ntiles) g = (int)ntiles;
    return g < 1 ? 1 : g;
}

hipError_t launch_merge_pass(const PassParams& p, int input_u16, int big_endian, int device, hipStream_t s) {
    if (p.ntiles == 0) return hipSuccess;
    if (!input_u16) {
        const void* fn = big_endian ? (const void*)merge_pass_kernel<uint8_t, true> : (const void*)merge_pass_kernel<uint8_t, false>;
        const int grid = grid_for(p.ntiles, device, fn, kThreads, big_endian ? 1 : 0);
        if (big_endian) hipLaunchKernelGGL((merge_pass_kernel<uint8_t, true>), dim3(grid), dim3(kThreads), 0, s, p);
        else hipLaunchKernelGGL((merge_pass_kernel<uint8_t, false>), dim3(grid), dim3(kThreads), 0, s, p);
        return hipGetLastError();
    }
    const bool lds = p.hbytes <= kHashLdsMax;
    const void* fn = lds ? (const void*)merge_tokens_kernel<true> : (const void*)merge_tokens_kernel<false>;
    const size_t smem = lds ? p.hbytes : 0;
    const int grid = grid_for_smem(p.ntiles, device, fn, kThreads, smem);
    if (lds) hipLaunchKernelGGL((merge_tokens_kernel<true>), dim3((unsigned)grid), dim3(kThreads), smem, s, p);
    else hipLaunchKernelGGL((merge_tokens_kernel<false>), dim3((unsigned)grid), dim3(kThreads), 0, s, p);
    return hipGetLastError();
}

hipError_t launch_scan_bytes(const PassParams& p, int mode, int live, int device, hipStream_t s) {
    if (p.ntiles == 0) return hipSuccess;
    using seg::scan_bytes_kernel;
    const void* fn = mode == 0 ? (const void*)scan_bytes_kernel<true, 0, false>
                     : mode == 1 ? (live ? (const void*)scan_bytes_kernel<true, 1, true> : (const void*)scan_bytes_kernel<true, 1, false>)
                                 : (live ? (const void*)scan_bytes_kernel<true, 2, true> : (const void*)scan_bytes_kernel<true, 2, false>);
    if (mode < 0 || mode > 2 || (mode == 0 && live)) return hipErrorInvalidValue;
    const int grid = grid_for(p.ntiles, device, fn, seg::kThreads, 4);
    const dim3 g((unsigned)grid), b(seg::kThreads);
    if (mode == 0) hipLaunchKernelGGL((scan_bytes_kernel<true, 0, false>), g, b, 0, s, p);
    else if (mode == 1 && live) hipLaunchKernelGGL((scan_bytes_kernel<true, 1, true>), g, b, 0, s, p);
    else if (mode == 1) hipLaunchKernelGGL((scan_bytes_kernel<true, 1, false>), g, b, 0, s, p);
    else if (live) hipLaunchKernelGGL((scan_bytes_kernel<true, 2, true>), g, b, 0, s, p);
    else hipLaunchKernelGGL((scan_bytes_kernel<true, 2, false>), g, b, 0, s, p);
    return hipGetLastError();
}

hipError_t launch_scan_tokens(const PassParams& p, int map_ready, int device, hipStream_t s) {
    if (p.n == 0) return hipSuccess;
    const uint64_t ranges = (p.n + kTokRange - 1) / kTokRange;
    if (!map_ready) hipLaunchKernelGGL(seg::chunk_map_kernel, dim3((unsigned)((ranges + 255) / 256)), dim3(256), 0, s, p);
    const bool lds = p.hbytes <= kHashLdsMax;
    const int mode = lds ? (p.hone ? 2 : 1) : 0;
    const void* fn = mode == 2 ? (const void*)seg::scan_tokens_kernel<2>
                     : mode == 1 ? (const void*)seg::scan_tokens_kernel<1> : (const void*)seg::scan_tokens_kernel<0>;
    const uint32_t ntiles = (uint32_t)((p.n + kTilePosTok - 1) / kTilePosTok);
    const int grid = grid_for(ntiles, device, fn, seg::kThreads, 5 + mode);
    const size_t smem = lds ? ((size_t)p.hbytes + 1023) & ~(size_t)1023 : 0;
    const dim3 g((unsigned)grid), b(seg::kThreads);
    if (mode == 2) hipLaunchKernelGGL((seg::scan_tokens_kernel<2>), g, b, smem, s, p);
    else if (mode == 1) hipLaunchKernelGGL((seg::scan_tokens_kernel<1>), g, b, smem, s, p);
    else hipLaunchKernelGGL((seg::scan_tokens_kernel<0>), g, b, 0, s, p);
    return hipGetLastError();
}

hipError_t launch_scan_fused(const PassParams& p, int device, hipStream_t s) {
    if (p.n == 0) return hipSuccess;
    if (p.hbytes > kHashLdsMax || p.cs < kMinChunkBytes || !p.fused_fail) return hipErrorInvalidValue;
    const int mode = p.hone ? 2 : 1;
    const void* fn = mode == 2 ? (const void*)seg::scan_tokens_kernel<2, true> : (const void*)seg::scan_tokens_kernel<1, true>;
    const uint32_t ntiles = (uint32_t)((p.n + kTilePosTok - 1) / kTilePosTok);
    const int grid = grid_for(ntiles, device, fn, seg::kThreads, 8 + mode);
    const size_t smem = ((size_t)p.hbytes + 1023) & ~(size_t)1023;
    const dim3 g((unsigned)grid), b(seg::kThreads);
    if (mode == 2) hipLaunchKernelGGL((seg::scan_tokens_kernel<2, true>), g, b, smem, s, p);
    else hipLaunchKernelGGL((seg::scan_tokens_kernel<1, true>), g, b, smem, s, p);
    return hipGetLastError();
}

hipError_t launch_basic_expand(const uint8_t* in, uint64_t n, uint8_t* out, hipStream_t s) {
    if (n == 0) return hipSuccess;
    uint64_t blocks = (n / 8 + 255) / 256;
    if (blocks < 1) blocks = 1;
    if (blocks > kBasicMaxBlocks) blocks = kBasicMaxBlocks;
    hipLaunchKernelGGL(basic_expand_kernel, dim3((unsigned)blocks), dim3(256), 0, s, in, n, out);
    return hipGetLastError();
}

hipError_t launch_chain_final(const uint64_t* tot, const uint32_t* done, const uint64_t* off1, uint64_t* chunk_off,
                              uint64_t nchunks, uint32_t k_last, uint64_t* tot_final, hipStream_t s) {
    const uint64_t blocks = chunk_off ? (nchunks + 1 + 255) / 256 : 1;
    hipLaunchKernelGGL(chain_final_kernel, dim3((unsigned)blocks), dim3(256), 0, s, tot, done, off1, chunk_off, nchunks,
                       k_last, tot_final);
    return hipGetLastError();
}

hipError_t launch_finish(const PassParams& p, int device, hipStream_t s) {
    if (p.nchunks == 0 || !p.fin_gate || p.nchunks > 0xFFFFFFFFull * 256u) return hipErrorInvalidValue;
    hipLaunchKernelGGL(finish_gate_kernel, dim3((unsigned)((p.nchunks + 255) / 256)), dim3(256), 0, s, p);
    const bool lds = p.hbytes <= kHashLdsMax;
    const int mode = lds ? (p.hone ? 2 : 1) : 0;
    const size_t smem = lds ? (size_t)p.hbytes : 0;
    const void* fn = mode == 2 ? (const void*)finish_chunks_kernel<2>
                     : mode == 1 ? (const void*)finish_chunks_kernel<1> : (const void*)finish_chunks_kernel<0>;
    const int grid = grid_for_smem((uint32_t)std::min<uint64_t>(p.nchunks, 0xFFFFFFFFull), device, fn, kFinThreads, smem);
    const dim3 g((unsigned)grid), b(kFinThreads);
    if (mode == 2) hipLaunchKernelGGL((finish_chunks_kernel<2>), g, b, smem, s, p);
    else if (mode == 1) hipLaunchKernelGGL((finish_chunks_kernel<1>), g, b, smem, s, p);
    else hipLaunchKernelGGL((finish_chunks_kernel<0>), g, b, 0, s, p);
    return hipGetLastError();
}

__device__ __forceinline__ uint32_t sp_lookup(const SparseParams& q, uint32_t key) {
    const uint2 x = q.hbuckets[bucket_hash(key, q.hmul1, q.hshift)];
    const uint2 y = q.hbuckets[bucket_hash(key, q.hmul2, q.hshift)];
    return (x.x == key ? x.y : 0u) | (y.x == key ? y.y : 0u);
}
__device__ __forceinline__ bool sp_bit(const uint32_t* b, uint64_t p) { return ((b[p >> 5] >> (p & 31u)) & 1u) != 0u; }
__device__ __forceinline__ int64_t sp_prev(const SparseParams& q, int64_t p) {
    for (--p; p >= 0 && sp_bit(q.holes, (uint64_t)p); --p) {}
    return p;
}
__device__ __forceinline__ uint64_t sp_next(const SparseParams& q, uint64_t p) {
    for (++p; p < q.n && sp_bit(q.holes, p); ++p) {}
    return p;
}
__device__ __forceinline__ uint32_t sp_key(const SparseParams& q, uint64_t a, uint64_t b) {
    return (uint32_t)q.tok[a] | ((uint32_t)q.tok[b] << 16);
}

__device__ __forceinline__ bool sp_gated(const SparseParams& q) { return q.gate && *q.gate != 0ull; }
__device__ __forceinline__ bool sp_compact_skip(const SparseParams& q, const uint32_t* nseeds0) {
    (void)nseeds0;
    return sp_gated(q) || (*q.flags & 2u) != 0u || (q.cond && *q.cond != 0u);
}

__global__ __launch_bounds__(1024) void sparse_sample_kernel(SparseParams q) {
    __shared__ uint32_t s_w[16];
    if (sp_gated(q)) return;
    for (uint32_t i = blockIdx.x * 1024u + threadIdx.x; i < q.zero16; i += kSparseSampleBlocks * 1024u)
        q.zero[i] = make_uint4(0u, 0u, 0u, 0u);
    const uint64_t n = *q.n_dev;
    const uint64_t p0 = n <= kSparseSample ? (uint64_t)blockIdx.x * 8192u
                                           : ((n - 8192u) / (kSparseSampleBlocks - 1u) * blockIdx.x) & ~7ull;
    const uint64_t i0 = p0 + 8ull * threadIdx.x;
    uint32_t t[9];
    if (i0 + 9 <= n) {
        const uint4 v = *reinterpret_cast<const uint4*>(q.tok + i0);
        const uint32_t w[4] = {v.x, v.y, v.z, v.w};
#pragma unroll
        for (int k = 0; k < 8; ++k) t[k] = (w[k >> 1] >> (16 * (k & 1))) & 0xFFFFu;
        t[8] = q.tok[i0 + 8];
    } else {
#pragma unroll
        for (int k = 0; k < 9; ++k) t[k] = i0 + k < n ? q.tok[i0 + k] : 0u;
    }
    uint32_t cnt = 0;
#pragma unroll
    for (int k = 0; k < 8; ++k)
        if (i0 + k + 1 < n) cnt += sp_lookup(q, t[k] | (t[k + 1] << 16)) >> 31;
#pragma unroll
    for (int d = 32; d >= 1; d >>= 1) cnt += (uint32_t)__shfl_xor((int)cnt, d, 64);
    if ((threadIdx.x & 63) == 0) s_w[threadIdx.x >> 6] = cnt;
    __syncthreads();
    if (threadIdx.x == 0) {
        uint32_t tot = 0;
#pragma unroll
        for (int k = 0; k < 16; ++k) tot += s_w[k];
        q.sample[blockIdx.x] = tot;
    }
}

constexpr uint32_t kListWords = 16 * 256, kListBlocks = 512;
__host__ __device__ __forceinline__ uint64_t sp_list_words(uint64_t nwords) {
    const uint64_t r = (nwords + (uint64_t)kListBlocks * kListWords - 1) / ((uint64_t)kListBlocks * kListWords);
    return (r ? r : 1ull) * kListWords;
}

constexpr uint64_t kDetectCsLds = 2048;
template <bool kLds>
__global__ __launch_bounds__(256) void sparse_detect_kernel(SparseParams qa) {
    extern __shared__ __attribute__((aligned(16))) uint32_t s_dyn[];
    if (sp_gated(qa)) return;
    SparseParams q = qa;
    q.n = *qa.n_dev;
    {
        const uint64_t sampled = q.n < kSparseSample ? q.n : kSparseSample;
        uint32_t smp = q.sample[threadIdx.x & 63];
#pragma unroll
        for (int d = 32; d >= 1; d >>= 1) smp += (uint32_t)__shfl_xor((int)smp, d, 64);
        if ((uint64_t)smp * q.n > (uint64_t)(q.cap / 2) * sampled) {
            if (blockIdx.x == 0 && threadIdx.x == 0) atomicOr(q.flags, 3u);
            return;
        }
    }
    const int lane = threadIdx.x & 63;
    const uint2* tab = q.hbuckets;
// ... 594 lines not shown
```

Measured before the change: 1974 GB/s.

## Templatize byte-scan tile geometry; use 3 sub-tiles with in-place prefetch for mode 0

The byte-scan kernel now takes the number of 16 KiB sub-tiles per tile as a template parameter. Mode 0 without live tracking runs 3 sub-tiles (48 KiB tiles) instead of 2. That mode also reuses a single register buffer: each sub-tile's input registers are refilled with the next tile's data as soon as phase 1 is done with them, and the forced-token raw bytes are reloaded from memory instead of read from the registers. Chunk-boundary arithmetic moves from tile units to sub-tile units, and workspace accounting is decoupled from the tile count. The goal is larger tiles per workgroup, which means fewer look-back and scheduling steps, without the register cost of double buffering. The costs are extra byte loads on forced positions, higher register pressure from the larger tile, and a risk of lower occupancy.

After: 2234 GB/s, median of 6. +13.2%, better.

```diff
diff --git a/blt_amd/_lib.py b/blt_amd/_lib.py
--- a/blt_amd/_lib.py
+++ b/blt_amd/_lib.py
@@ -85,6 +85,7 @@
     "blt_debug_set_inject": (ctypes.c_uint32, [ctypes.c_uint32]),
     "blt_debug_last_u16_passes": (ctypes.c_uint32, []),
     "blt_debug_last_scan_passes": (ctypes.c_uint32, []),
+    "blt_debug_last_byte_tile": (ctypes.c_uint32, []),
     "blt_debug_set_u16_chain": (ctypes.c_int, [ctypes.c_int]),
     "blt_debug_set_fused_only": (ctypes.c_int, [ctypes.c_int]),
     "blt_debug_set_shared_contexts": (None, [ctypes.c_int]),
diff --git a/blt_amd/csrc/blt_host.cpp b/blt_amd/csrc/blt_host.cpp
--- a/blt_amd/csrc/blt_host.cpp
+++ b/blt_amd/csrc/blt_host.cpp
@@ -522,6 +522,7 @@
 thread_local uint32_t t_last_u16_passes = 0;
 thread_local uint32_t t_last_scan_passes = 0;
 thread_local uint32_t t_last_fused = 0;
+thread_local uint32_t t_last_byte_tile = 0;
 
 inline uint64_t up16(uint64_t x) { return (x + 15) & ~15ull; }
 inline uint64_t up256(uint64_t x) { return (x + 255) & ~255ull; }
@@ -624,7 +625,8 @@
              uint64_t out_cap, uint64_t* chunk_off, bool ws_zeroed = false, const Chain* chain = nullptr,
              bool tok_scan = false, U16Run* run = nullptr) {
     const bool columnar = !in_u16 && cs >= blt::kMinChunkBytes && h->byte_mode >= 0 && be;
-    const uint64_t tile = columnar ? blt::kTilePosBytes
+    const int byte_live = (chain && h->live_first) ? 1 : 0;
+    const uint64_t tile = columnar ? blt::scan_bytes_tile(h->byte_mode, byte_live)
                                    : in_u16 ? (tok_scan ? blt::kTilePosTok : blt::kTilePosU16) : blt::kTilePos;
     const uint64_t ntiles = (n + tile - 1) / tile;
     if (ntiles > 0xFFFFFFFFull) return fail(BLT_E_INVALID_INPUT, "input too large");
@@ -662,9 +664,9 @@
     p.hbytes = (uint32_t)(h->hwords.size() * sizeof(uint32_t));
     p.hone = h->hone ? 1u : 0u;
     p.cs_magic = cs ? ~0ull / cs : 0;
-    if (cs && cs % blt::kTilePosBytes == 0 && cs / blt::kTilePosBytes < (1ull << 31)) {
-        p.cs_tiles = (uint32_t)(cs / blt::kTilePosBytes);
-        p.cs_tiles_magic = p.cs_tiles > 1 ? (uint32_t)(0xFFFFFFFFull / p.cs_tiles) : 0u;
+    if (cs && cs % blt::kSubPosBytes == 0 && n / blt::kSubPosBytes < (1ull << 31) - 8) {
+        p.cs_subs = (uint32_t)std::min<uint64_t>(cs / blt::kSubPosBytes, 0x7FFFFFFFull);
+        p.cs_subs_magic = p.cs_subs > 1 ? (uint32_t)(0xFFFFFFFFull / p.cs_subs) : 0u;
     }
     p.allm = h->allmerge ? 1u : 0u;
     p.mark = h->mark | (h->mark << 16);
@@ -690,7 +692,10 @@
         run->map_ready = scan16 && chain->next_scan;
     }
     p.ws_check = (ws_zeroed && !in_u16 && !chain) ? 1u : 0u;
-    if (columnar) HIP_TRY(blt::launch_scan_bytes(p, h->byte_mode, (chain && h->live_first) ? 1 : 0, dev, s));
+    if (columnar) {
+        HIP_TRY(blt::launch_scan_bytes(p, h->byte_mode, byte_live, dev, s));
+        t_last_byte_tile = (uint32_t)tile;
+    }
     else if (scan16) {
         HIP_TRY(blt::launch_scan_tokens(p, ready ? 1 : 0, dev, s));
         ++t_last_scan_passes;
@@ -1809,6 +1814,7 @@
 
 uint32_t blt_debug_last_u16_passes(void) { return t_last_u16_passes; }
 uint32_t blt_debug_last_scan_passes(void) { return t_last_scan_passes; }
+uint32_t blt_debug_last_byte_tile(void) { return t_last_byte_tile; }
 
 int blt_debug_inject_device_error(const blt_bpe* h, void* d_ws, void* stream) {
     if (!h) return fail(BLT_E_INVALID_INPUT, "null handle");
diff --git a/blt_amd/csrc/bpe_kernels.h b/blt_amd/csrc/bpe_kernels.h
--- a/blt_amd/csrc/bpe_kernels.h
+++ b/blt_amd/csrc/bpe_kernels.h
@@ -10,6 +10,7 @@
 constexpr uint64_t kTilePosTok = 32768;
 constexpr uint64_t kTokRange = 1024;
 constexpr uint64_t kTilePosBytes = 32768;
+constexpr uint64_t kSubPosBytes = 16384;
 constexpr uint64_t kMinChunkBytes = 4096;
 constexpr uint64_t kCtlBytes = 64;
 constexpr uint32_t kCtlLeft = 15;
@@ -45,8 +46,8 @@
     uint64_t* status_zero;
     uint32_t tick;
     uint64_t cs_magic;
-    uint32_t cs_tiles;
-    uint32_t cs_tiles_magic;
+    uint32_t cs_subs;
+    uint32_t cs_subs_magic;
     uint32_t allm;
     uint32_t mark;
     uint32_t* sticky;
@@ -60,6 +61,8 @@
 
 hipError_t launch_merge_pass(const PassParams& p, int input_u16, int big_endian, int device, hipStream_t s);
 hipError_t launch_scan_bytes(const PassParams& p, int mode, int live, int device, hipStream_t s);
+constexpr int scan_bytes_subtiles(int mode, int live) { return (mode == 0 && !live) ? 3 : 2; }
+constexpr uint64_t scan_bytes_tile(int mode, int live) { return (uint64_t)scan_bytes_subtiles(mode, live) * kSubPosBytes; }
 constexpr uint32_t kDoneBytePass = 0x80000000u;
 hipError_t launch_scan_tokens(const PassParams& p, int map_ready, int device, hipStream_t s);
 hipError_t launch_scan_fused(const PassParams& p, int device, hipStream_t s);
diff --git a/blt_amd/csrc/bpe_kernels.hip b/blt_amd/csrc/bpe_kernels.hip
--- a/blt_amd/csrc/bpe_kernels.hip
+++ b/blt_amd/csrc/bpe_kernels.hip
@@ -640,6 +640,7 @@
 constexpr int kThreads = 1024;
 constexpr int kWaves = kThreads / 64;
 constexpr int kS = 2;
+constexpr int kSMax = 3;
 constexpr int kLdPol = 2, kStPol = 2;
 constexpr uint32_t kWavePos = 64u * 16u;
 constexpr uint64_t kSubPos = (uint64_t)kWaves * kWavePos;
@@ -647,11 +648,13 @@
 constexpr int kStageWave = 1536;
 constexpr int kLbWin = 1;
 constexpr uint32_t kNone = 0xFFFFFFFFu;
-static_assert(kSubPos * kS == kTilePosBytes, "tile geometry");
+static_assert(kSubPos == kSubPosBytes, "sub-tile geometry");
 static_assert(kWavePos <= kMinChunkBytes, "at most one chunk end per wave sub-tile");
-static_assert(kGroups <= 64, "one lane per group in the tile resolve");
+static_assert(kSMax * kWaves <= 64, "one lane per group in the tile resolve");
+static_assert((uint64_t)kSMax * kSubPos < 65536u, "a tile's token counts fit the packed 16-bit scan");
 static_assert(kStageWave % 16 == 0, "stage alignment");
-static_assert((uint64_t)kS * kSubPos == kTilePosBytes, "tile = kS sub-tiles");
+static_assert((uint64_t)kS * kSubPos == kTilePosBytes, "the default tile is the workspace's accounting unit");
+static_assert(scan_bytes_subtiles(0, 0) <= kSMax && scan_bytes_subtiles(1, 1) == kS, "instantiated geometries");
 
 __device__ __forceinline__ uint32_t uni(uint32_t v) { return (uint32_t)__builtin_amdgcn_readfirstlane((int)v); }
 __device__ __forceinline__ uint64_t uni64(uint64_t v) {
@@ -704,20 +707,25 @@
     uint64_t k0;
 };
 
-constexpr uint32_t kFarPos = 2u * (uint32_t)kTilePosBytes;
+template <int NS>
+constexpr uint32_t kTileBytes = (uint32_t)NS * (uint32_t)kSubPos;
+template <int NS>
+constexpr uint32_t kFarPos = 2u * kTileBytes<NS>;
+template <int NS>
 __device__ __forceinline__ TInfo tile_info(const PassParams& p, uint32_t T) {
     TInfo t;
-    const uint64_t tile0 = (uint64_t)T * kTilePosBytes;
+    const uint64_t tile0 = (uint64_t)T * kTileBytes<NS>;
     const uint64_t left = p.n > tile0 ? p.n - tile0 : 0;
     t.rn = (uint32_t)(left > 0x7FFFFFFFull ? 0x7FFFFFFFull : left);
-    if (p.cs_tiles) {
-        const uint32_t d = p.cs_tiles;
-        uint32_t q = d == 1u ? T : __umulhi(T, p.cs_tiles_magic);
-        uint32_t r = T - q * d;
+    if (p.cs_subs) {
+        const uint32_t d = p.cs_subs;
+        const uint32_t S = (uint32_t)NS * T;
+        uint32_t q = d == 1u ? S : __umulhi(S, p.cs_subs_magic);
+        uint32_t r = S - q * d;
         if (r >= d) { q += 1u; r -= d; }
         if (r >= d) { q += 1u; r -= d; }
-        const uint32_t left_tiles = r ? d - r : 0u;
-        t.bge = left_tiles > 2u ? kFarPos : left_tiles * (uint32_t)kTilePosBytes;
+        const uint32_t left_subs = r ? d - r : 0u;
+        t.bge = left_subs > 2u * (uint32_t)NS ? kFarPos<NS> : left_subs * (uint32_t)kSubPos;
         t.k0 = (uint64_t)q + (r ? 1u : 0u);
         return t;
     }
@@ -727,7 +735,7 @@
     if (r >= cs) { q += 1; r -= cs; }
     if (r >= cs) { q += 1; r -= cs; }
     const uint64_t d = r ? cs - r : 0;
-    t.bge = (uint32_t)(d > kFarPos ? kFarPos : d);
+    t.bge = (uint32_t)(d > kFarPos<NS> ? kFarPos<NS> : d);
     t.k0 = q + (r ? 1u : 0u);
     return t;
 }
@@ -781,16 +789,17 @@
     }
 }
 
-template <bool kBE, int kMode, bool kLive>
-__device__ __forceinline__ void phase1_tile(uint32_t tab, const uint32_t (&x)[kS][4], const uint32_t (&nxt)[kS],
-                                            const TInfo& ti, uint32_t cs32, uint32_t wave, int lane,
-                                            TileState& st, uint32_t (*wfn)[4], uint32_t allm, uint32_t mark,
-                                            uint64_t* sub = nullptr) {
+template <bool kBE, int kMode, bool kLive, int NS, bool kXEarly, typename XDead>
+__device__ __forceinline__ void phase1_tile(const PassParams& p, uint32_t T, uint32_t tab, const uint32_t (&x)[NS][4],
+                                            const uint32_t (&nxt)[NS], const TInfo& ti, uint32_t cs32, uint32_t wave,
+                                            int lane, TileStateT<NS>& st, uint32_t (*wfn)[4], uint32_t allm,
+                                            uint32_t mark, uint64_t* sub, XDead&& x_dead) {
     static_assert(kBE, "the byte pass writes big-endian tokens");
     static_assert(kMode >= 0 && kMode <= 2 && !(kLive && kMode == 0), "phase-1 mode");
-    uint32_t m[kS];
-#pragma unroll
-    for (int j = 0; j < kS; ++j) {
+    static_assert(!kXEarly || kMode == 0, "modes 1 and 2 read x for their merge test");
+    uint32_t m[NS];
+#pragma unroll
+    for (int j = 0; j < NS; ++j) {
         const uint32_t nbw = (uint32_t)__builtin_amdgcn_update_dpp((int)nxt[j], (int)x[j][0], 0x130, 0xF, 0xF, false);
 #pragma unroll
         for (int h = 0; h < 8; ++h) {
@@ -808,6 +817,7 @@
             }
             st.v[j][h] = __builtin_amdgcn_perm(vb, va, 0x05040100u);
         }
+        if constexpr (kXEarly) x_dead(j);
         uint32_t m32 = 0;
 #pragma unroll
         for (int h = 0; h < 8; ++h) {
@@ -830,7 +840,7 @@
     }
     uint32_t bnext = ti.bge;
 #pragma unroll
-    for (int j = 0; j < kS; ++j) {
+    for (int j = 0; j < NS; ++j) {
         const uint32_t wrel = (uint32_t)j * (uint32_t)kSubPos + wave * kWavePos;
         while (bnext <= wrel) bnext += cs32;
         const uint32_t rem = ti.rn > wrel ? ti.rn - wrel : 0u;
@@ -841,16 +851,28 @@
             const uint32_t vmask = r >= 16 ? 0xFFFFu : (r <= 0 ? 0u : ((1u << r) - 1u));
             uint32_t mm = m[j] & ((vmask >> 1) | (r > 16 ? 0x8000u : 0u));
             uint32_t forced = (r >= 1 && r <= 16) ? (1u << (r - 1)) : 0u;
+            uint32_t e = 16u;
             if (has_end) {
-                const uint32_t e = bnext - 1u - wrel - l16;
+                e = bnext - 1u - wrel - l16;
                 if (e < 16u) { mm &= ~(1u << e); forced |= 1u << e; }
             }
             if (__ballot(forced != 0)) {
+                uint32_t b1 = 0, b2 = 0;
+                if constexpr (kXEarly) {
+                    const uint64_t tile0 = (uint64_t)T * kTileBytes<NS>;
+                    const __amdgpu_buffer_rsrc_t rs =
+                        rsrc_at(reinterpret_cast<const uint8_t*>(KARG(in)) + tile0, p.n > tile0 ? p.n - tile0 : 0);
+                    const uint32_t o = wrel + l16, oob = 0x80000000u;
+                    b1 = (uint32_t)__builtin_amdgcn_raw_buffer_load_b8(rs, (int)((r >= 1 && r <= 16) ? o + (uint32_t)(r - 1) : oob), 0, 0);
+                    b2 = (uint32_t)__builtin_amdgcn_raw_buffer_load_b8(rs, (int)(e < 16u ? o + e : oob), 0, 0);
+                }
 #pragma unroll
                 for (int h = 0; h < 8; ++h) {
                     const uint32_t xw = x[j][h >> 1];
-                    const uint32_t raw = __builtin_amdgcn_perm(xw, xw, kBE ? ((h & 1) ? 0x030C020Cu : 0x010C000Cu)
-                                                                           : ((h & 1) ? 0x0C030C02u : 0x0C010C00u));
+                    const uint32_t raw = kXEarly ? ((((uint32_t)(2 * h) == e ? b2 : b1) & 0xFFu) << 8) |
+                                                       ((((uint32_t)(2 * h + 1) == e ? b2 : b1) & 0xFFu) << 24)
+                                                 : __builtin_amdgcn_perm(xw, xw, kBE ? ((h & 1) ? 0x030C020Cu : 0x010C000Cu)
+                                                                                     : ((h & 1) ? 0x0C030C02u : 0x0C010C00u));
                     const uint32_t fm = (((forced >> (2 * h)) & 1u) ? 0x0000FFFFu : 0u) |
                                         (((forced >> (2 * h + 1)) & 1u) ? 0xFFFF0000u : 0u);
                     st.v[j][h] = (st.v[j][h] & ~fm) | (raw & fm);
@@ -862,11 +884,12 @@
             st.mv[j] = m[j] | 0xFFFF0000u;
         }
     }
+    if constexpr (!kXEarly) x_dead(0);
     uint32_t wlive = 0;
     if (kLive) {
         uint32_t lv = 0;
 #pragma unroll
-        for (int j = 0; j < kS; ++j) {
+        for (int j = 0; j < NS; ++j) {
             uint32_t low32 = 0;
 #pragma unroll
             for (int h = 0; h < 8; ++h) low32 |= (pk_nz(st.v[j][h] & 0x00FF00FFu) ^ 0x00010001u) << (2 * h);
@@ -878,7 +901,7 @@
         asm volatile("s_waitcnt lgkmcnt(0)" ::: "memory");
         sub[0] = __builtin_amdgcn_s_memtime();
     }
-    lane_wave_fns<kS>(m, wave, lane, st, wfn, wlive);
+    lane_wave_fns<NS>(m, wave, lane, st, wfn, wlive);
     if (sub) {
         asm volatile("s_waitcnt lgkmcnt(0)" ::: "memory");
         sub[1] = __builtin_amdgcn_s_memtime();
@@ -1216,9 +1239,11 @@
     uint32_t gb, wcnt;
 };
 
+template <int NS>
 __device__ __forceinline__ void emit_tile(const PassParams& p, uint32_t Tp, const TInfo& ti, uint32_t cs32,
-                                          uint32_t wave, int lane, const TileState& st, const uint32_t (*gin)[4],
+                                          uint32_t wave, int lane, const TileStateT<NS>& st, const uint32_t (*gin)[4],
                                           uint32_t C, uint64_t O, uint8_t* stg, bool has_coff) {
+    constexpr bool kInline = NS > kS;
     uint8_t* out = reinterpret_cast<uint8_t*>(KARG(out));
     const uint64_t out_cap = KARG(out_cap);
     const uint64_t obase = (2ull * O) & ~15ull;
@@ -1227,10 +1252,26 @@
     const uint32_t stg_lds = lds_addr(stg);
     uint32_t cnext = ti.bge;
     uint64_t kc = ti.k0;
-    SparseRange sr[kS];
-    bool sparse[kS];
-#pragma unroll
-    for (int j = 0; j < kS; ++j) {
+    SparseRange sr[NS];
+    bool sparse[NS];
+    auto emit_sparse = [&](int j) {
+        const uint32_t two = (sr[j].gb & 15u) + 2u * sr[j].wcnt <= (uint32_t)kStageWave ? 0u : 1u;
+        const uint32_t off32 = two ? uni(lane_u32(sr[j].lane_off, 32)) : 0u;
+        for (uint32_t part = 0; part <= two; ++part) {
+            const uint32_t base = part ? off32 : 0u;
+            const uint32_t cnt = two ? (part ? sr[j].wcnt - off32 : off32) : sr[j].wcnt;
+            const uint32_t gbp = sr[j].gb + 2u * base;
+            if (!two || ((uint32_t)lane >> 5) == part) {
+                stage_b16(st.v[j], sr[j].L, stg_lds + (gbp & 15u) + 2u * (sr[j].lane_off - base));
+            }
+            const CopyPart cp = {gbp & ~15u, gbp & 15u, (gbp & 15u) + 2u * cnt};
+            CopyData<> d;
+            copy_read(stg, cp, lane, d);
+            copy_store(ro, cp, lane, d);
+        }
+    };
+#pragma unroll
+    for (int j = 0; j < NS; ++j) {
         const uint32_t g = (uint32_t)j * kWaves + wave;
         const uint32_t wrel = (uint32_t)j * (uint32_t)kSubPos + wave * kWavePos;
         const uint32_t cg = uni(gin[g][C]);
@@ -1260,45 +1301,33 @@
         sr[j].lane_off = lane_off;
         sr[j].gb = gb;
         sr[j].wcnt = uni(lane_u32(lane_off + __popc(L), 63));
-    }
-    auto fits = [&](int j) { return (sr[j].gb & 15u) + 2u * sr[j].wcnt <= (uint32_t)kStageWave; };
-#pragma unroll
-    for (int j = 0; j < kS; ++j) {
-        if (!sparse[j]) continue;
-        const uint32_t two = fits(j) ? 0u : 1u;
-        const uint32_t off32 = two ? uni(lane_u32(sr[j].lane_off, 32)) : 0u;
-        for (uint32_t part = 0; part <= two; ++part) {
-            const uint32_t base = part ? off32 : 0u;
-            const uint32_t cnt = two ? (part ? sr[j].wcnt - off32 : off32) : sr[j].wcnt;
-            const uint32_t gbp = sr[j].gb + 2u * base;
-            if (!two || ((uint32_t)lane >> 5) == part) {
-                stage_b16(st.v[j], sr[j].L, stg_lds + (gbp & 15u) + 2u * (sr[j].lane_off - base));
-            }
-            const CopyPart cp = {gbp & ~15u, gbp & 15u, (gbp & 15u) + 2u * cnt};
-            CopyData<> d;
-            copy_read(stg, cp, lane, d);
-            copy_store(ro, cp, lane, d);
-        }
-    }
-}
-
+        if constexpr (kInline) emit_sparse(j);
+    }
+    if constexpr (!kInline) {
+#pragma unroll
+        for (int j = 0; j < NS; ++j)
+            if (sparse[j]) emit_sparse(j);
+    }
+}
+
+template <int NS>
 __device__ __forceinline__ void load_tile(const PassParams& p, uint32_t Tn, uint32_t wave, int lane,
-                                          uint32_t (&x)[kS][4], uint32_t (&nxt)[kS]) {
+                                          uint32_t (&x)[NS][4], uint32_t (&nxt)[NS]) {
     const uint8_t* in = reinterpret_cast<const uint8_t*>(KARG(in));
-    const uint64_t tile0 = (uint64_t)Tn * kTilePosBytes;
+    const uint64_t tile0 = (uint64_t)Tn * kTileBytes<NS>;
     const uint64_t left = p.n > tile0 ? p.n - tile0 : 0;
     const __amdgpu_buffer_rsrc_t r = rsrc_at(in + tile0, left);
     const __amdgpu_buffer_rsrc_t rd = rsrc_at(in + tile0, left & ~3ull);
     const uint32_t rn = (uint32_t)(left > 0x7FFFFFFFull ? 0x7FFFFFFFull : left);
 #pragma unroll
-    for (int j = 0; j < kS; ++j) {
+    for (int j = 0; j < NS; ++j) {
         const uint32_t wrel = (uint32_t)j * (uint32_t)kSubPos + wave * kWavePos;
         const auto v = __builtin_amdgcn_raw_buffer_load_b128(rd, (int)wrel + 16 * lane, 0, kLdPol);
         x[j][0] = v[0]; x[j][1] = v[1]; x[j][2] = v[2]; x[j][3] = v[3];
         nxt[j] = (uint32_t)__builtin_amdgcn_raw_buffer_load_b32(rd, (int)(wrel + kWavePos), 0, 0);
     }
 #pragma unroll
-    for (int j = 0; j < kS; ++j) {
+    for (int j = 0; j < NS; ++j) {
         const uint32_t wrel = (uint32_t)j * (uint32_t)kSubPos + wave * kWavePos;
         if (rn > wrel && rn - wrel < kWavePos + 16u) {
             nxt[j] = (uint32_t)__builtin_amdgcn_raw_buffer_load_b8(r, (int)(wrel + kWavePos), 0, 0);
@@ -1311,6 +1340,29 @@
                          << (8 * b);
                 x[j][q] = d;
             }
+        }
+    }
+}
+
+template <int NS>
+__device__ __forceinline__ void load_sub(const PassParams& p, uint32_t Tn, __amdgpu_buffer_rsrc_t rd, uint32_t rn, int j,
+                                         uint32_t wave, int lane, uint32_t (&x)[4], uint32_t& nxt) {
+    const uint32_t wrel = (uint32_t)j * (uint32_t)kSubPos + wave * kWavePos;
+    const auto v = __builtin_amdgcn_raw_buffer_load_b128(rd, (int)wrel + 16 * lane, 0, kLdPol);
+    x[0] = v[0]; x[1] = v[1]; x[2] = v[2]; x[3] = v[3];
+    nxt = (uint32_t)__builtin_amdgcn_raw_buffer_load_b32(rd, (int)(wrel + kWavePos), 0, 0);
+    if (rn > wrel && rn - wrel < kWavePos + 16u) {
+        const uint64_t tile0 = (uint64_t)Tn * kTileBytes<NS>;
+        const __amdgpu_buffer_rsrc_t r =
+            rsrc_at(reinterpret_cast<const uint8_t*>(KARG(in)) + tile0, p.n > tile0 ? p.n - tile0 : 0);
+        nxt = (uint32_t)__builtin_amdgcn_raw_buffer_load_b8(r, (int)(wrel + kWavePos), 0, 0);
+#pragma unroll
+        for (int q = 0; q < 4; ++q) {
+            uint32_t d = 0;
+#pragma unroll
+            for (int b = 0; b < 4; ++b)
+                d |= (uint32_t)__builtin_amdgcn_raw_buffer_load_b8(r, (int)wrel + 16 * lane + 4 * q + b, 0, 0) << (8 * b);
+            x[q] = d;
         }
     }
 }
@@ -1341,12 +1393,16 @@
     }
 }
 
-template <bool kBE, int kMode, bool kLive>
+template <bool kBE, int kMode, bool kLive, int NS>
 __global__ __launch_bounds__(kThreads) void scan_bytes_kernel(PassParams p) {
+    constexpr int kG = NS * kWaves;
+    constexpr bool kInPlace = NS > kS;
+    static_assert(!kInPlace || kMode == 0, "in-place refill: phase 1 must not read x after its lookups");
+    constexpr bool kLbFresh = kMode != 0 || kInPlace;
     __shared__ __attribute__((aligned(16))) uint16_t s_tab[kSelfEntries];
     __shared__ __attribute__((aligned(16))) uint8_t s_stage[kWaves][kStageWave];
-    __shared__ __attribute__((aligned(16))) uint32_t s_wfn[kRing][kGroups][4];
-    __shared__ uint32_t s_gin[kRing][kGroups][4];
+    __shared__ __attribute__((aligned(16))) uint32_t s_wfn[kRing][kG][4];
+    __shared__ uint32_t s_gin[kRing][kG][4];
     __shared__ uint32_t s_tfn[kRing][4];
     __shared__ uint64_t s_O[kRing];
     __shared__ uint32_t s_C[kRing];
@@ -1361,7 +1417,8 @@
     const uint32_t wave = uni((uint32_t)tid >> 6);
     const uint64_t n = p.n;
     const uint32_t ntiles = p.ntiles;
-    const uint32_t cs32 = (uint32_t)(p.cs > kFarPos ? kFarPos : p.cs);
+    const uint32_t cs32 = (uint32_t)(p.cs > kFarPos<NS> ? kFarPos<NS> : p.cs);
+    const uint32_t ws_words = NS == kS ? ntiles : (uint32_t)((n + kTilePosBytes - 1) / kTilePosBytes);
     const uint32_t allm = uni(p.allm), mark = uni(p.mark);
     const bool has_coff = p.chunk_off != nullptr;
 
@@ -1394,28 +1451,35 @@
     uint32_t T = uni(s_tk[kRing - 2]);
     uint32_t Tp = kNone;
     uint32_t Tq = uni(s_tk[kRing - 1]);
-    if (ws_refused(p, ntiles, cover)) T = kNone;
+    if (ws_refused(p, ws_words, cover)) T = kNone;
     if (T >= ntiles || Tq >= ntiles) Tq = kNone;
     TInfo ti = {}, tip = {};
-    if (T < ntiles) ti = tile_info(p, T);
+    if (T < ntiles) ti = tile_info<NS>(p, T);
     __syncthreads();
 
-    uint32_t xa[kS][4], xb[kS][4];
-    uint32_t na[kS], nb[kS];
-    if (T < ntiles) load_tile(p, T, wave, lane, xa, na);
-    TileState sa, sb;
+    uint32_t xa[NS][4], xb[NS][4];
+    uint32_t na[NS], nb[NS];
+    if (T < ntiles) load_tile<NS>(p, T, wave, lane, xa, na);
+    TileStateT<NS> sa, sb;
     uint64_t lbs[kLbWin];
     uint32_t it = 0;
 
-    auto step = [&](uint32_t (&x)[kS][4], uint32_t (&nxt)[kS], uint32_t (&xq)[kS][4], uint32_t (&nxtq)[kS],
-                    TileState& sc, const TileState& sp) {
+    auto step = [&](uint32_t (&x)[NS][4], uint32_t (&nxt)[NS], uint32_t (&xq)[NS][4], uint32_t (&nxtq)[NS],
+                    TileStateT<NS>& sc, const TileStateT<NS>& sp) {
         const uint32_t slot = it & (kRing - 1), pslot = (it - 1) & (kRing - 1);
         uint64_t stamp[7], sub[2] = {0, 0};
         const bool stamping = kTiming && p.debug != nullptr;
         if (stamping) stamp[0] = __builtin_amdgcn_s_memtime();
         __builtin_amdgcn_s_waitcnt(0x0F70);
         if (stamping) stamp[1] = __builtin_amdgcn_s_memtime();
-        if (Tq < ntiles) load_tile(p, Tq, wave, lane, xq, nxtq);
+        if (!kInPlace && Tq < ntiles) load_tile<NS>(p, Tq, wave, lane, xq, nxtq);
+        uint64_t q0 = 0, qleft = 0;
+        if (kInPlace && Tq < ntiles) {
+            q0 = (uint64_t)Tq * kTileBytes<NS>;
+            qleft = n > q0 ? n - q0 : 0;
+        }
+        const __amdgpu_buffer_rsrc_t rdq = rsrc_at(reinterpret_cast<const uint8_t*>(KARG(in)) + q0, qleft & ~3ull);
+        const uint32_t rnq = (uint32_t)(qleft > 0x7FFFFFFFull ? 0x7FFFFFFFull : qleft);
         uint32_t tk = kNone;
         if (tid == kTkTid && Tq < ntiles) tk = atomicAdd(p.ctl, 1u);
         asm volatile("" ::: "memory");
@@ -1423,8 +1487,10 @@
         bool lbw = wave == 0;
         if (T < ntiles) {
             if (wave >= (uint32_t)kPrioP1Wave) __builtin_amdgcn_s_setprio(kPrioP1);
-            phase1_tile<kBE, kMode, kLive>(tab, x, nxt, ti, cs32, wave, lane, sc, s_wfn[slot], allm, mark,
-                                           stamping ? sub : nullptr);
+            phase1_tile<kBE, kMode, kLive, NS, kInPlace>(
+                p, T, tab, x, nxt, ti, cs32, wave, lane, sc, s_wfn[slot], allm, mark, stamping ? sub : nullptr, [&](int j) {
+                    if constexpr (kInPlace) load_sub<NS>(p, Tq, rdq, rnq, j, wave, lane, xq[j], nxtq[j]);
+                });
             __builtin_amdgcn_s_setprio(0);
             uint32_t old = 0;
             if (lane == 0)
@@ -1432,7 +1498,7 @@
             old = uni(old);
             lbw = old == (uint32_t)kWaves * (it / kRing);
             if (old == (uint32_t)kWaves * (it / kRing + 1u) - 1u) {
-                resolve_tile<kGroups, kLive, kMode != 0>(p, T, lane, s_wfn[slot], s_gin[slot], s_tfn[slot]);
+                resolve_tile<kG, kLive, kLbFresh>(p, T, lane, s_wfn[slot], s_gin[slot], s_tfn[slot]);
                 if (lane == 0) lds_release(&s_rdone, it + 1u);
                 if (stamping && lane == 0) p.debug[4ull * ntiles + 4ull * T] = __builtin_amdgcn_s_memrealtime();
             }
@@ -1443,16 +1509,16 @@
             uint32_t C = 1u, how = 0xFFFFu, spins = 0, bad = 0, live = 0;
             uint64_t O = 0ull;
             const bool lb = Tp > 0;
-            if (lb) lb_issue<kMode != 0>(p, (int64_t)Tp - 1, lane, lbs);
+            if (lb) lb_issue<kLbFresh>(p, (int64_t)Tp - 1, lane, lbs);
             const uint64_t rt_snap = stamping ? __builtin_amdgcn_s_memrealtime() : 0;
             wait_ge(p, &s_rdone, it);
             const uint32_t tfl = uni(s_tfn[pslot][0]), tf1 = uni(s_tfn[pslot][1]);
             const uint32_t tf0 = tfl & 1u, tf2 = uni(s_tfn[pslot][2]), tf3 = uni(s_tfn[pslot][3]);
-            if (lb) lb_finish<kMode != 0>(p, Tp, lane, lbs, C, O, how, spins, live, kTiming ? &bad : nullptr);
+            if (lb) lb_finish<kLbFresh>(p, Tp, lane, lbs, C, O, how, spins, live, kTiming ? &bad : nullptr);
             live |= (tfl >> 1) & 1u;
             if (lane == 0) {
                 const uint64_t end = O + (C == 1u ? tf3 : tf2);
-                if (C > 1u || O > (uint64_t)Tp * kTilePosBytes || end > n) {
+                if (C > 1u || O > (uint64_t)Tp * kTileBytes<NS> || end > n) {
                     if (C <= 1u) record_error(p, 4u, Tp, 0xFFu, O, end, C);
                     O = 0; C = 2u;
                 }
@@ -1490,7 +1556,7 @@
             if (wave >= (uint32_t)kPrioEmWave) __builtin_amdgcn_s_setprio(kPrioEm);
             const uint32_t Cp = uni(s_C[pslot]);
             if (Cp <= 1u)
-                emit_tile(p, Tp, tip, cs32, wave, lane, sp, s_gin[pslot], Cp, uni64(s_O[pslot]), s_stage[wave], has_coff);
+                emit_tile<NS>(p, Tp, tip, cs32, wave, lane, sp, s_gin[pslot], Cp, uni64(s_O[pslot]), s_stage[wave], has_coff);
             __builtin_amdgcn_s_setprio(0);
         }
         if (stamping) stamp[5] = __builtin_amdgcn_s_memtime();
@@ -1517,7 +1583,7 @@
             if (Tr >= ntiles) Tr = kNone;
         }
         tip = ti;
-        if (Tq < ntiles) ti = tile_info(p, Tq);
+        if (Tq < ntiles) ti = tile_info<NS>(p, Tq);
         Tp = T;
         T = Tq;
         Tq = Tr;
@@ -1525,13 +1591,13 @@
     };
     for (;;) {
         if (!(T < ntiles || Tp < ntiles)) break;
-        step(xa, na, xb, nb, sa, sb);
+        if constexpr (kInPlace) step(xa, na, xa, na, sa, sb); else step(xa, na, xb, nb, sa, sb);
         if (!(T < ntiles || Tp < ntiles)) break;
-        step(xb, nb, xa, na, sb, sa);
+        if constexpr (kInPlace) step(xa, na, xa, na, sb, sa); else step(xb, nb, xa, na, sb, sa);
     }
     if (wg_rec && lane == 0)
         atomicMax(reinterpret_cast<unsigned long long*>(wg_rec + 2), (unsigned long long)__builtin_amdgcn_s_memrealtime());
-    self_reset(p, ntiles, &s_tkdone);
+    self_reset(p, ws_words, &s_tkdone);
 }
 
 constexpr int kSt = (int)(kTilePosTok / kTokRange) / kWaves;
@@ -2592,17 +2658,20 @@
 hipError_t launch_scan_bytes(const PassParams& p, int mode, int live, int device, hipStream_t s) {
     if (p.ntiles == 0) return hipSuccess;
     using seg::scan_bytes_kernel;
-    const void* fn = mode == 0 ? (const void*)scan_bytes_kernel<true, 0, false>
-                     : mode == 1 ? (live ? (const void*)scan_bytes_kernel<true, 1, true> : (const void*)scan_bytes_kernel<true, 1, false>)
-                                 : (live ? (const void*)scan_bytes_kernel<true, 2, true> : (const void*)scan_bytes_kernel<true, 2, false>);
     if (mode < 0 || mode > 2 || (mode == 0 && live)) return hipErrorInvalidValue;
+    constexpr int kS0 = scan_bytes_subtiles(0, 0), kSx = seg::kS;
+    if (scan_bytes_subtiles(mode, live) != (mode == 0 ? kS0 : kSx)) return hipErrorInvalidValue;
+    if (p.ntiles != (p.n + scan_bytes_tile(mode, live) - 1) / scan_bytes_tile(mode, live)) return hipErrorInvalidValue;
+    const void* fn = mode == 0 ? (const void*)scan_bytes_kernel<true, 0, false, kS0>
+                     : mode == 1 ? (live ? (const void*)scan_bytes_kernel<true, 1, true, kSx> : (const void*)scan_bytes_kernel<true, 1, false, kSx>)
+                                 : (live ? (const void*)scan_bytes_kernel<true, 2, true, kSx> : (const void*)scan_bytes_kernel<true, 2, false, kSx>);
     const int grid = grid_for(p.ntiles, device, fn, seg::kThreads, 4);
     const dim3 g((unsigned)grid), b(seg::kThreads);
-    if (mode == 0) hipLaunchKernelGGL((scan_bytes_kernel<true, 0, false>), g, b, 0, s, p);
-    else if (mode == 1 && live) hipLaunchKernelGGL((scan_bytes_kernel<true, 1, true>), g, b, 0, s, p);
-    else if (mode == 1) hipLaunchKernelGGL((scan_bytes_kernel<true, 1, false>), g, b, 0, s, p);
-    else if (live) hipLaunchKernelGGL((scan_bytes_kernel<true, 2, true>), g, b, 0, s, p);
-    else hipLaunchKernelGGL((scan_bytes_kernel<true, 2, false>), g, b, 0, s, p);
+    if (mode == 0) hipLaunchKernelGGL((scan_bytes_kernel<true, 0, false, kS0>), g, b, 0, s, p);
+    else if (mode == 1 && live) hipLaunchKernelGGL((scan_bytes_kernel<true, 1, true, kSx>), g, b, 0, s, p);
+    else if (mode == 1) hipLaunchKernelGGL((scan_bytes_kernel<true, 1, false, kSx>), g, b, 0, s, p);
+    else if (live) hipLaunchKernelGGL((scan_bytes_kernel<true, 2, true, kSx>), g, b, 0, s, p);
+    else hipLaunchKernelGGL((scan_bytes_kernel<true, 2, false, kSx>), g, b, 0, s, p);
     return hipGetLastError();
 }
 
```
